# lmcinnes/enstop

Hardware: AMD Instinct MI355X
Metric: EM iterations/sec (higher is better)
Workload: dtype f32; 1 GPU; 1M x 100k, 100M nnz; corpus=independent Zipf tokens (SURVEY 8d), nnz=100435863, k=64, schedule=fused, parallelism=single fit

## Files before the change

### enstop_amd/csrc/plsa_hip.hip

```cpp
#include <hip/hip_runtime.h>
#include <hipcub/hipcub.hpp>
#include <rccl/rccl.h>

#include <algorithm>
#include <cmath>
#include <cstdarg>
#include <cstdio>
#include <cstdlib>
#include <cstring>
#include <memory>
#include <mutex>
#include <string>
#include <thread>
#include <type_traits>
#include <vector>

#include "../../include/plsa_hip.h"
#include "../../include/plsa_hip_diag.h"
#include "../../include/plsa_hip_members.h"
#include "../../include/plsa_hip_metrics.h"
#include "../../include/plsa_hip_blocked.h"
#include "../../include/plsa_hip_embed.h"
#include "../../include/plsa_hip_nmf.h"
#include "../../include/plsa_hip_score.h"
#include "../../include/plsa_hip_tempered.h"
#include "../../include/plsa_hip_online.h"
#include "mt_jump.hpp"
#include "plsa_embed_kernels.hpp"
#include "plsa_init_kernels.hpp"
#include "plsa_init_plan.hpp"
#include "plsa_kernels.hpp"
#include "plsa_launch_plan.hpp"
#include "plsa_member_kernels.hpp"
#include "plsa_metric_kernels.hpp"
#include "plsa_nmf_kernels.hpp"
#include "plsa_ref_kernels.hpp"
#include "plsa_synth.hpp"

using plsa::i64;

namespace {

thread_local std::string g_err;


struct DevBuf {
    void *p = nullptr;
    size_t cap = 0;
    bool borrowed = false;
    DevBuf() = default;
    DevBuf(DevBuf &&o) noexcept { swap(o); }
    DevBuf &operator=(DevBuf &&o) noexcept { DevBuf(std::move(o)).swap(*this); return *this; }
    void swap(DevBuf &o) noexcept { std::swap(p, o.p); std::swap(cap, o.cap); std::swap(borrowed, o.borrowed); }
    ~DevBuf() { if (p && !borrowed) (void)hipFree(p); }
    void release() { if (!borrowed) *this = DevBuf(); }
    void borrow(void *q, size_t bytes) { *this = DevBuf(); p = q; cap = q ? bytes : 0; borrowed = q != nullptr; }
    template <class T> T *as() const { return reinterpret_cast<T *>(p); }
};

template <class H, hipError_t (*Destroy)(H)>
struct Handle {
    H h = nullptr;
    Handle() = default;
    Handle(Handle &&o) noexcept { std::swap(h, o.h); }
    Handle &operator=(Handle &&o) noexcept { Handle(std::move(o)).swap(*this); return *this; }
    void swap(Handle &o) noexcept { std::swap(h, o.h); }
    ~Handle() { if (h) (void)Destroy(h); }
    operator H() const { return h; }
};
using Stream = Handle<hipStream_t, hipStreamDestroy>;
using Event = Handle<hipEvent_t, hipEventDestroy>;

struct HostFree { void operator()(void *p) const { (void)hipHostFree(p); } };
template <class T> using Pinned = std::unique_ptr<T[], HostFree>;
template <class T> hipError_t host_alloc(Pinned<T> &h, size_t count) {
    h.reset();
    void *q = nullptr;
    const hipError_t e = hipHostMalloc(&q, sizeof(T) * count, hipHostMallocDefault);
    h.reset(static_cast<T *>(q));
    return e;
}

template <class T> struct Derived {
    bool valid = false;
    void invalidate() { valid = false; }
    void drop() { static_cast<T &>(*this) = T{}; }
};

struct Timed {
    int name_id;
    Event a, b;
};

}

struct plsa_ctx {
    int device = 0;
    Stream stream;
    Stream stream2;
    hipStream_t ls = nullptr;
    Event ev_fork, ev_join;
    Event ev_row, ev_tail;
    bool overlap = true;
    double overlap_full_limit = 2e9;
    std::string err;
    hipDeviceProp_t prop;
    int grid_cap = 2048;

    i64 bn = 0, bm = 0, bnnz = 0;
    DevBuf b_indptr, b_col, b_val;
    bool active_is_base = true;
    i64 n = 0, m = 0, nnz = 0;
    DevBuf a_indptr, a_col, a_val;
    const int *indptr = nullptr, *col = nullptr;
    const float *val = nullptr;
    struct RowIndex : Derived<RowIndex> { DevBuf ids; } rowidx;

    struct Csc : Derived<Csc> {
        DevBuf colptr, row, val, pos, item_first, item_col, item_start, item_end, item_order, heavy_cols;
        DevBuf item_rec;
        DevBuf xcd_lo;
        bool balanced = false;
        int seg = 256, n_heavy = 0;
        i64 n_items = 0;
    } csc;
    int seg_override = 0, struct_lpn = 0;
    int struct_row_lpn = 0;
    DevBuf partial;
    bool use_item_order = true, xcd_split = true;
    bool packed = true;
    struct PackedStream : Derived<PackedStream> {
        DevBuf buf;
        bool ok = false;
        int state() const { return !valid ? -1 : (ok ? 1 : 0); }
    } pk_csr, pk_csc;
    DevBuf pk_count;
    int chunks_per_lane = 2;
    int row_lpn = 1, row_ch = 1;
    bool row_shape_8x2 = true;
    bool p_lent = false;
    int e_rows = -1;
    int mt_streams = 256;
    i64 mt_min_blocks = 4096;
    int heavy_items = 32;

    bool force_wide = false;
    struct RowItems : Derived<RowItems> {
        DevBuf first, row, start;
        bool use = false;
        int seg = 64;
        i64 n = 0;
    } ritems;
    int rseg_override = 0, ritems_mode = -1;
    DevBuf rpartial;

    struct EItems : Derived<EItems> { DevBuf row, start; int seg = 0; i64 n = 0; } eitems;
    int eseg_override = -1;

    bool sort_rows = true;
    struct RowOrder : Derived<RowOrder> {
        DevBuf ids;
        int range = 0;
    } roworder;
    i64 syn_n = 0; int syn_k0 = 0; double syn_alpha = 0.0; uint64_t syn_seed = 0;
    bool row_xcd = false;

    int k = 0, kp = 0, lpn = 1, ch = 1;
    DevBuf U[3], Vt[3], Vacc;
    bool rot3 = false;
    int speculate = -1;
    Event ev_ll;
    int cu = 0, cv = 0;
    i64 fac_n = 0, fac_m = 0;
    DevBuf P;
    struct PState : Derived<PState> {} p_state;
    bool ref_sums = false, ref_ll = false;
    DevBuf ref_terms;
    int ref_chain_mode = 0;
    bool ref_pairs_off = false;
    DevBuf ref_csum, ref_pairs, ref_exps, ref_pairs2, ref_exps2, ref_stats, ref_ll_neg;
    struct RefTileSums : Derived<RefTileSums> {
        DevBuf sums;
        const float *sw = nullptr;
        int tj = 0;
    } ref_tsum;
    const float *ref_e_sw = nullptr;
    bool ref_e_no_sums = false;
    struct RefHeavy : Derived<RefHeavy> { DevBuf cols; int n = 0, min = 0; } ref_heavy;
    int64_t p_budget = 0;
    struct RefBlocks : Derived<RefBlocks> {
        std::vector<i64> doc, ent;
        int64_t budget = 0;
        int kp = 0;
        i64 largest = 0;
        int blocks() const { return (int)doc.size() - 1; }
    } ref_blocks;
    struct PBlockInfo { int64_t budget = 0; int blocks = 0; int64_t largest = 0, p_bytes = 0; } p_block_info;
    Pinned<unsigned long long> h_ref_stats;
    Event ev_ref_stats;
    bool ref_stats_pending = false;
    unsigned long long ref_slow_total = 0, ref_chunks_total = 0;
    int placement_candidates = 4, placement_tried = 0;
    double placement_gbps[2] = {0.0, 0.0};
    size_t p_shift = 0;

    DevBuf sw, ll_partials, ll_out, colsum_partials, norm_pwz, norm_pdz, tmp0, tmp1, tmp2, cubtmp;
    DevBuf mt_seq;
    bool mt_chain = false;
    DevBuf mt_words, mt_state, mt_fin, mt_poly;
    Pinned<double> h_ll;

    DevBuf colsum_rows, colsum_rows2;
    DevBuf metric_mask, metric_small;
    struct Nmf { DevBuf raw, guarded, slabs, obj, out; } nmf;
    struct Score { DevBuf indptr, col, val, flag, out; } score;
    struct Tempered {
        DevBuf U, Vt, snapU, snapVt;
        bool have_snap = false;
        i64 snap_n = 0, snap_m = 0;
        int snap_k = 0;
    } tempered;
    DevBuf t_end;
    bool pipeline = true;
    bool graph = false;
    int order_band = -1;
    int balance = -1;
    bool bal_have_frac = false;
    double bal_frac[9] = {0, 0, 0, 0, 0, 0, 0, 0, 0};
    int bal_lo[9] = {0, 0, 0, 0, 0, 0, 0, 0, 0};
    i64 bal_chunks = -1;
    int bal_launches = 0;
    double bal_end_us[8] = {0, 0, 0, 0, 0, 0, 0, 0};
    int small_grid = 0;
    int colsum_rows_used = 0;
    struct FitInfo {
        int fused = 0, pipelined = 0, speculated = 0, graph_launches = 0;
        int tail = 0;
        int two_stage = 0;
        int xcd_split = 0;
    } fit_info;

    ncclComm_t comm = nullptr;
    int comm_rank = 0, comm_world = 1;
    bool sharded = false;
    bool sw_resident = false;
    i64 sw_n = 0;
    DevBuf sw_res;
    DevBuf comm_send, comm_recv, comm_small, comm_stack;
    Pinned<float> comm_host;
    size_t comm_host_cap = 0;

    bool timing = false;
    std::vector<std::string> names;
    std::vector<Timed> timed;
    std::vector<Event> pool;
    std::vector<double> acc_ms;
    std::vector<i64> acc_n;
};

namespace {

inline float *p_base(plsa_ctx *c) { return reinterpret_cast<float *>(reinterpret_cast<char *>(c->P.p) + c->p_shift); }

int fail(plsa_ctx *c, const char *fmt, ...) {
    char buf[512];
    va_list ap;
    va_start(ap, fmt);
    vsnprintf(buf, sizeof buf, fmt, ap);
    va_end(ap);
    if (c) c->err = buf; else g_err = buf;
    return 1;
}

#define HIPCHK(c, expr)                                                                            \
    do {                                                                                           \
        hipError_t e_ = (expr);                                                                    \
        if (e_ != hipSuccess)                                                                      \
            return fail((c), "%s failed: %s (%s:%d)", #expr, hipGetErrorString(e_), __FILE__,      \
                        __LINE__);                                                                 \
    } while (0)

#define CHK(expr)                                                                                  \
    do {                                                                                           \
        int r_ = (expr);                                                                           \
        if (r_) return r_;                                                                         \
    } while (0)
// ... 267 lines not shown

int launch_check(plsa_ctx *c, const char *what) {
    hipError_t e = hipGetLastError();
    if (e != hipSuccess) return fail(c, "launch of %s failed: %s", what, hipGetErrorString(e));
    return 0;
}

inline int out_u(const plsa_ctx *c) { return c->rot3 ? (c->cu + 1) % 3 : 1 - c->cu; }
inline int out_v(const plsa_ctx *c) { return c->rot3 ? (c->cv + 1) % 3 : 1 - c->cv; }

int grid_for(plsa_ctx *c, i64 work_items, int items_per_block) {
    return plsa::plan::grid_for(work_items, items_per_block, c->grid_cap);
}

}

#include "plsa_structures.hpp"

namespace {

int upload_sw(plsa_ctx *c, const float *sw, const float **d_sw) {
    *d_sw = nullptr;
    if (!sw) {
        if (c->sw_resident) {
            if (c->sw_n != c->n) return fail(c, "resident sample weights were set for %lld documents, the active matrix has %lld",
                                              (long long)c->sw_n, (long long)c->n);
            *d_sw = c->sw_res.as<float>();
        }
        return 0;
    }
    CHK(ensure(c, c->sw, sizeof(float) * (size_t)c->n));
    HIPCHK(c, hipMemcpyAsync(c->sw.p, sw, sizeof(float) * (size_t)c->n, hipMemcpyHostToDevice, c->stream));
    HIPCHK(c, hipStreamSynchronize(c->stream));
    *d_sw = c->sw.as<float>();
    return 0;
}

int need_factors(plsa_ctx *c) {
    if (c->k <= 0 || !c->U[0].p || !c->Vt[0].p) return fail(c, "factors not set (call plsa_set_factors)");
    if (c->n <= 0) return fail(c, "no corpus uploaded");
    if (c->fac_n != c->n || c->fac_m != c->m)
        return fail(c, "factors were set for a %lld x %lld matrix but the active matrix is %lld x %lld "
                       "(call plsa_set_factors after plsa_upload_csr / plsa_bootstrap)",
                    (long long)c->fac_n, (long long)c->fac_m, (long long)c->n, (long long)c->m);
    return 0;
}

template <class Fn> void with_flag(bool v, Fn &&fn) { if (v) fn(std::true_type{}); else fn(std::false_type{}); }
template <bool V, class Fn> void with_flag(std::integral_constant<bool, V> v, Fn &&fn) { fn(v); }

int ensure_p(plsa_ctx *c, i64 rows) {
    {
        const size_t need = sizeof(float) * (size_t)(rows + 64) * (size_t)c->kp;
        size_t free_b = 0, total_b = 0;
        if (!c->P.borrowed && c->P.cap < need && hipMemGetInfo(&free_b, &total_b) == hipSuccess && free_b + c->P.cap < need)
            return fail(c, c->ref_sums ? "the reference arithmetic (PLSA_REFERENCE_SUMS) stores P(z|w,d) like the reference does: %.1f GB needed, "
                                         "%.1f GB of HBM free -- at this size only the default arithmetic is available, or this one block "
                                         "of documents at a time (plsa_set_p_budget / p_budget=, plsa_fit and plsa_refit)"
                                       : "materialising P(z|w,d) needs %.1f GB but only %.1f GB of HBM are free; use the fused "
                           "schedule (PLSA_FUSED), which never stores it, or tile the documents (plsa_em_accumulate_materialised)", need / 1e9, (free_b + c->P.cap) / 1e9);
    }
    if (c->P.borrowed || c->p_lent) {
        const size_t need = sizeof(float) * (size_t)(rows + 64) * (size_t)c->kp;
        if (c->P.cap < need)
            return fail(c, c->P.borrowed ? "the borrowed P(z|w,d) buffer holds %.2f GB, this matrix needs %.2f GB (plsa_p_borrow)"
                                         : "the P(z|w,d) buffer lent out by plsa_p_reserve holds %.2f GB, this matrix needs %.2f GB: it cannot "
                                           "grow while other contexts hold its address (end the loans, then plsa_release_scratch)",
                        c->P.cap / 1e9, need / 1e9);
        c->p_shift = 0;
    } else
    {
        const char *s1 = getenv("PLSA_P_SLACK_MB"), *s2 = getenv("PLSA_P_OFFSET_KB");
        const bool budgeted = c->ref_sums && c->p_budget > 0;
        const size_t slack = s1 && !budgeted ? (size_t)atoll(s1) << 20 : 0;
        c->p_shift = s2 && !budgeted ? (size_t)atoll(s2) * 1024 : 0;
        CHK(ensure_best_placement(c, c->P, sizeof(float) * (size_t)(rows + 64) * (size_t)c->kp + std::max(slack, c->p_shift),
                                  budgeted ? 1 : c->placement_candidates, c->placement_gbps, &c->placement_tried));
    }
    return 0;
}

}

#include "plsa_ref.hpp"

namespace {

int run_e_step(plsa_ctx *c, float thresh) {
    c->ref_tsum.invalidate();
    CHK(ensure_p(c, c->nnz));
    if (c->ref_sums) return run_ref_e_step(c, thresh);
    bool e_rows = c->e_rows < 0 ? (double)c->nnz * c->kp >= 1e8 : c->e_rows != 0;
    if (e_rows) {
        const int eseg = plsa::plan::e_item_len(c->lpn, c->eseg_override);
        CHK(ensure_eitems(c, eseg));
        const bool items = eseg > 0 && c->eitems.n > 0;
        const int grid = grid_for(c, items ? c->eitems.n : c->n, 256 / c->lpn);
        const int *order = nullptr;
        if (!items) CHK(ensure_roworder(c, &order));
        CHK(dispatch_shape(c, [&](auto S) {
            Scope s(c, "k_e_step");
            auto go = [&](auto TN) {
                hipLaunchKernelGGL((plsa::k_e_step_rows<decltype(S), decltype(TN)::value>), dim3(grid), dim3(256), 0, c->stream,
                                   c->indptr, c->col, (int)c->n, order, c->U[c->cu].as<float>(), c->Vt[c->cv].as<float>(),
                                   p_base(c), c->kp, thresh, items ? c->eitems.row.as<int>() : nullptr,
                                   items ? c->eitems.start.as<int>() : nullptr, eseg, c->eitems.n);
            };
            if (thresh < plsa::TINY_THRESH) go(std::true_type{}); else go(std::false_type{});
        }));
    } else {
        CHK(ensure_rowidx(c));
        const i64 tiles = (c->nnz + 63) / 64;
        const int grid = grid_for(c, tiles, 4);
        CHK(dispatch_shape(c, [&](auto S) {
            Scope s(c, "k_e_step");
            auto go = [&](auto TN) {
                hipLaunchKernelGGL((plsa::k_e_step<decltype(S), decltype(TN)::value>), dim3(grid), dim3(256), 0, c->stream,
                                   c->rowidx.ids.as<int>(), c->col, c->nnz, c->U[c->cu].as<float>(),
                                   c->Vt[c->cv].as<float>(), p_base(c), c->kp, thresh);
            };
            if (thresh < plsa::TINY_THRESH) go(std::true_type{}); else go(std::false_type{});
        }));
    }
    CHK(launch_check(c, "k_e_step"));
    c->p_state.valid = true;
    return 0;
}

template <class Sh, class FromP, class Fn>
void select_row_pass(bool packed, FromP from_p, bool want_ll, bool tiny, Fn &&fn) {
    with_flag(from_p, [&](auto FP) {
        if constexpr (decltype(FP)::value) fn(Sh{}, FP, std::false_type{}, std::false_type{});
        else with_flag(want_ll, [&](auto LL) {
            with_flag(tiny, [&](auto TN) { if (packed) fn(plsa::Packed<Sh>{}, FP, LL, TN); else fn(Sh{}, FP, LL, TN); });
        });
    });
}

template <class Sh, class FromP, class Timed, class Fn>
void select_col_pass(bool packed, FromP from_p, Timed timed, bool tiny, Fn &&fn) {
    with_flag(from_p, [&](auto FP) {
        with_flag(timed, [&](auto TM) {
            if constexpr (decltype(FP)::value) fn(Sh{}, FP, TM, std::false_type{});
            else with_flag(tiny, [&](auto TN) { if (packed) fn(plsa::Packed<Sh>{}, FP, TM, TN); else fn(Sh{}, FP, TM, TN); });
        });
    });
}

struct RowLaunch {
    plsa::plan::RowPass plan;
    bool items, packed, xcd_rows;
    const int *indptr, *colidx;
    const float *vals;
    const int *order;
    const int *ritem_row, *ritem_start, *ritem_first;
    float *rpartial;
    double *ll_partials;
    i64 n_ritems;
    int rseg;
};

int prepare_row_pass(plsa_ctx *c, bool from_p, bool want_ll, RowLaunch &r) {
    CHK(ensure_ritems(c));
    r.items = c->ritems.use && c->ritems.n > 0;
    r.xcd_rows = !r.items && !from_p && c->sort_rows && row_xcd_range(c) > 0;
    r.plan = plsa::plan::row_pass(c->n, c->ritems.n, r.items, c->row_lpn, c->grid_cap, r.xcd_rows);
    r.order = nullptr;
    if (!r.items) CHK(ensure_roworder(c, &r.order));
    if (r.items) CHK(ensure(c, c->rpartial, sizeof(float) * (size_t)c->ritems.n * c->kp));
    if (want_ll) CHK(ensure(c, c->ll_partials, sizeof(double) * (size_t)r.plan.grid));
    if (!from_p) CHK(ensure_packed_csr(c));
    r.packed = !from_p && c->packed && c->pk_csr.ok;
    r.indptr = c->indptr; r.colidx = r.packed ? c->pk_csr.buf.as<int>() : c->col; r.vals = c->val;
    r.ritem_row = r.items ? c->ritems.row.as<int>() : nullptr;
    r.ritem_start = r.items ? c->ritems.start.as<int>() : nullptr;
    r.ritem_first = r.items ? c->ritems.first.as<int>() : nullptr;
    r.rpartial = r.items ? c->rpartial.as<float>() : nullptr;
    r.ll_partials = c->ll_partials.as<double>();
    r.n_ritems = c->ritems.n; r.rseg = c->ritems.seg;
    return 0;
}

int run_row_pass(plsa_ctx *c, bool from_p, bool want_ll, const float *d_sw, float thresh,
                 float *d_norm_pdz, int *ll_blocks) {
    RowLaunch r;
    CHK(prepare_row_pass(c, from_p, want_ll, r));
    CHK(dispatch_shape_row(c, [&](auto S) {
        using Sh = decltype(S);
        const float *U = c->U[c->cu].as<float>(), *Vt = c->Vt[c->cv].as<float>();
        float *Un = c->U[out_u(c)].as<float>();
        const int n = (int)c->n, kp = c->kp;
        select_row_pass<Sh>(r.packed, from_p, want_ll, thresh < plsa::TINY_THRESH, [&](auto SS, auto FP, auto LL, auto TN) {
            Scope s(c, from_p ? "k_row_pass<P>" : want_ll ? "k_row_pass<fused,LL>" : "k_row_pass<fused>");
            hipLaunchKernelGGL((plsa::k_row_pass<decltype(SS), decltype(FP)::value, decltype(LL)::value, decltype(TN)::value>),
                               dim3(r.plan.grid), dim3(256), 0, c->ls, r.indptr, r.colidx, r.vals, n, r.order, U, Vt, p_base(c), Un,
                               d_sw, d_norm_pdz, kp, thresh, r.ll_partials, r.ritem_row, r.ritem_start, r.rseg, r.n_ritems,
                               r.rpartial, r.xcd_rows ? 1 : 0);
        });
        if (r.items) {
            Scope s(c, "k_row_reduce");
            hipLaunchKernelGGL((plsa::k_row_reduce<Sh>), dim3(r.plan.reduce_grid), dim3(256), 0, c->ls,
                               r.ritem_first, n, r.rpartial, Un, d_norm_pdz, kp);
        }
    }));
    CHK(launch_check(c, "k_row_pass"));
    if (ll_blocks) *ll_blocks = r.plan.grid;
    return 0;
}

struct ColLaunch {
    plsa::plan::ColPass plan;
    bool packed;
    int xcd_split;
    const int4 *item_rec;
    i64 n_items;
    const int *csc_row, *csc_pos;
    const float *csc_val;
    float *partial;
    double *colsum_rows, *colsum_rows2;
    float *norm_pwz;
    const int *item_first, *heavy_cols;
    int n_heavy, heavy_items;
};

int prepare_col_pass(plsa_ctx *c, bool from_p, ColLaunch &l) {
    CHK(from_p ? ensure_csc(c) : ensure_packed_csc(c));
    l.packed = !from_p && c->packed && c->pk_csc.ok;
    l.plan = plsa::plan::col_pass(c->csc.n_items, c->m, c->lpn, c->csc.n_heavy, c->grid_cap);
    l.xcd_split = plsa::plan::xcd_split(c->xcd_split, l.plan.n_chunks, c->n, c->kp) ? 1 : 0;
    CHK(ensure(c, c->partial, sizeof(float) * (size_t)std::max<i64>(c->csc.n_items, 1) * c->kp));
    CHK(ensure(c, c->colsum_rows, sizeof(double) * (size_t)std::max(l.plan.n_chunks, 1) * c->kp));
    CHK(ensure(c, c->norm_pwz, sizeof(float) * (size_t)c->kp));
    if (l.plan.norm_blocks) CHK(ensure(c, c->colsum_rows2, sizeof(double) * (size_t)l.plan.norm_blocks * c->kp));
    l.item_rec = c->csc.item_rec.as<int4>(); l.n_items = c->csc.n_items;
    l.csc_row = l.packed ? c->pk_csc.buf.as<int>() : c->csc.row.as<int>();
    l.csc_pos = c->csc.pos.as<int>(); l.csc_val = c->csc.val.as<float>();
    l.partial = c->partial.as<float>(); l.norm_pwz = c->norm_pwz.as<float>();
    l.colsum_rows = c->colsum_rows.as<double>(); l.colsum_rows2 = c->colsum_rows2.as<double>();
    l.item_first = c->csc.item_first.as<int>(); l.heavy_cols = c->csc.heavy_cols.as<int>();
    l.n_heavy = c->csc.n_heavy; l.heavy_items = c->heavy_items;
    return 0;
}

int run_col_pass(plsa_ctx *c, bool from_p, const float *d_sw, float thresh, int parts = 3) {
    ColLaunch l;
    CHK(prepare_col_pass(c, from_p, l));
    int rc = 0;
    CHK(dispatch_shape_gather(c, table_is_wide(c, c->n), [&](auto S) {
        using Sh = decltype(S);
        constexpr int GPB = 256 / Sh::LPN;
        const int n_chunks = l.plan.n_chunks, kp = c->kp;
        if (parts & 1) {
            c->fit_info.xcd_split = l.xcd_split;
            const size_t smem = sizeof(double) * (size_t)GPB * kp;
            auto launch = [&](bool timed) -> int {
                int grid = plsa::plan::col_grid(c->bal_lo, n_chunks, l.xcd_split != 0);
                if (c->small_grid > 0 && (double)c->nnz * kp < c->overlap_full_limit)
                    grid = std::min(grid, c->small_grid * c->prop.multiProcessorCount);
                Scope s(c, from_p ? "k_col_pass<P>" : "k_col_pass<fused>");
                const int *lo = c->csc.xcd_lo.as<int>();
                const float *U = c->U[c->cu].as<float>(), *Vt = c->Vt[c->cv].as<float>();
                unsigned long long *te = c->t_end.as<unsigned long long>();
                select_col_pass<Sh>(l.packed, from_p, timed, thresh < plsa::TINY_THRESH, [&](auto SS, auto FP, auto TM, auto TN) {
                    hipLaunchKernelGGL((plsa::k_col_pass<decltype(SS), decltype(FP)::value, decltype(TM)::value, decltype(TN)::value>),
                                       dim3(grid), dim3(256), smem, c->ls, l.item_rec, l.n_items, lo, l.csc_row, l.csc_val, l.csc_pos,
                                       U, Vt, p_base(c), d_sw, l.partial, kp, thresh, l.xcd_split, l.colsum_rows, te);
                });
                return launch_check(c, "k_col_pass");
            };
            rc = ensure_balance(c, n_chunks, l.xcd_split != 0, launch);
            if (rc) return;
            rc = launch(false);
            if (rc) return;
            c->colsum_rows_used = n_chunks;
        }
        if (parts & 2) {
            Scope s(c, "k_col_reduce");
            hipLaunchKernelGGL((plsa::k_col_reduce<Sh>), dim3(l.plan.reduce_grid), dim3(256), GPB * kp * sizeof(float), c->ls,
                               l.item_first, (int)c->m, l.heavy_items, l.heavy_cols, l.n_heavy, l.partial, c->Vacc.as<float>(), kp);
        }
    }));
    if (rc) return rc;
    CHK(launch_check(c, "k_col_pass"));
    return 0;
}

int run_v_normalise(plsa_ctx *c) {
    if (c->sharded && c->comm) {
        Scope s(c, "rccl_allreduce_accumulator");
        NCCLCHK(c, ncclAllReduce(c->Vacc.p, c->Vacc.p, (size_t)c->m * c->kp, ncclFloat, ncclSum, c->comm, c->ls));
    }
    const int nb = (int)std::min<i64>(plsa::NORM_BLOCKS, std::max<i64>(1, c->m));
    CHK(ensure(c, c->colsum_partials, sizeof(double) * (size_t)nb * c->kp));
    {
        Scope s(c, "k_colsum_partial");
        hipLaunchKernelGGL(plsa::k_colsum_partial, dim3(nb), dim3(256), 256 * sizeof(double), c->ls,
                           c->Vacc.as<float>(), (int)c->m, c->kp, c->colsum_partials.as<double>());
    }
    CHK(ensure(c, c->norm_pwz, sizeof(float) * (size_t)c->kp));
    {
        Scope s(c, "k_colsum_final");
        hipLaunchKernelGGL(plsa::k_colsum_final, dim3(1), dim3(256), 0, c->ls,
                           c->colsum_partials.as<double>(), nb, c->kp, c->norm_pwz.as<float>());
    }
    {
        Scope s(c, "k_v_normalise");
        const i64 total4 = c->m * c->kp / 4;
        hipLaunchKernelGGL(plsa::k_v_normalise, dim3(grid_for(c, total4, 256)), dim3(256),
                           c->kp * sizeof(float), c->ls, c->Vacc.as<float>(),
                           c->Vt[out_v(c)].as<float>(), (int)c->m, c->kp, c->norm_pwz.as<float>());
    }
    CHK(launch_check(c, "k_v_normalise"));
    return 0;
}

int run_col_tail(plsa_ctx *c) {
    if (c->sharded) {
        c->fit_info.tail = 2;
        c->fit_info.two_stage = 0;
        CHK(run_col_pass(c, false, nullptr, 0.f, 2));
        return run_v_normalise(c);
    }
    ColLaunch l;
    CHK(prepare_col_pass(c, true, l));
    c->fit_info.tail = 1;
    c->fit_info.two_stage = l.plan.norm_blocks > 0;
    if (c->colsum_rows_used <= 0) return fail(c, "internal: column tail without a column pass");
    const double *rows_in = l.colsum_rows;
    int n_rows = l.plan.n_chunks;
    if (l.plan.norm_blocks) {
        Scope s(c, "k_norm_reduce");
        hipLaunchKernelGGL(plsa::k_norm_reduce, dim3(l.plan.norm_blocks), dim3(256), 0, c->ls, rows_in, n_rows, c->kp,
                           l.colsum_rows2);
        rows_in = l.colsum_rows2;
        n_rows = l.plan.norm_blocks;
    }
    {
        Scope s(c, "k_colsum_final");
        hipLaunchKernelGGL(plsa::k_colsum_final, dim3(1), dim3(256), 0, c->ls, rows_in, n_rows, c->kp, l.norm_pwz);
    }
    CHK(dispatch_shape(c, [&](auto S) {
        using Sh = decltype(S);
        constexpr int GPB = 256 / Sh::LPN;
        Scope s(c, "k_col_reduce_norm");
        hipLaunchKernelGGL((plsa::k_col_reduce_norm<Sh>), dim3(l.plan.reduce_grid), dim3(256),
                           sizeof(float) * (size_t)(GPB + 1) * c->kp, c->ls, l.item_first, (int)c->m, l.heavy_items, l.heavy_cols,
                           l.n_heavy, l.partial, l.norm_pwz, c->Vt[out_v(c)].as<float>(), c->kp);
    }));
    return launch_check(c, "k_col_reduce_norm");
}

int finish_ll(plsa_ctx *c, int blocks, double *out) {
    CHK(ensure(c, c->ll_out, sizeof(double)));
    {
        Scope s(c, "k_ll_final");
        hipLaunchKernelGGL(plsa::k_ll_final, dim3(1), dim3(256), 0, c->stream,
                           c->ll_partials.as<double>(), blocks, c->ll_out.as<double>());
    }
    CHK(launch_check(c, "k_ll_final"));
    if (c->sharded && c->comm)
        NCCLCHK(c, ncclAllReduce(c->ll_out.p, c->ll_out.p, 1, ncclDouble, ncclSum, c->comm, c->stream));
    HIPCHK(c, hipMemcpyAsync(c->h_ll.get(), c->ll_out.p, sizeof(double), hipMemcpyDeviceToHost, c->stream));
    if (!out) return hipEventRecord(c->ev_ll, c->stream) == hipSuccess ? 0 : fail(c, "event record failed");
    HIPCHK(c, hipStreamSynchronize(c->stream));
    *out = c->h_ll[0];
    return 0;
}

int wait_ll(plsa_ctx *c, double *out) {
    HIPCHK(c, hipEventSynchronize(c->ev_ll));
    *out = c->h_ll[0];
    return 0;
}

int run_loglik(plsa_ctx *c, const float *d_sw, double *out) {
    if (c->ref_ll) return run_ref_loglik(c, d_sw, out);
    const int grid = grid_for(c, c->n, 256 / c->lpn);
    const int *order = nullptr;
    CHK(ensure_roworder(c, &order));
    CHK(ensure(c, c->ll_partials, sizeof(double) * (size_t)grid));
    CHK(dispatch_shape(c, [&](auto S) {
        Scope s(c, "k_loglik");
        hipLaunchKernelGGL((plsa::k_loglik<decltype(S)>), dim3(grid), dim3(256), 0, c->stream, c->indptr,
                           c->col, c->val, (int)c->n, order, c->U[c->cu].as<float>(),
                           c->Vt[c->cv].as<float>(), d_sw, c->kp, c->ll_partials.as<double>());
    }));
    CHK(launch_check(c, "k_loglik"));
    return finish_ll(c, grid, out);
}

int run_m_step_from_p(plsa_ctx *c, const float *d_sw, bool update_v, float *d_norm_pdz) {
    if (!c->p_state.valid) return fail(c, "plsa_m_step: no P(z|w,d) on the device (run plsa_e_step or plsa_set_p)");
    if (c->ref_sums) return run_ref_m_step(c, d_sw, update_v, d_norm_pdz);
    CHK(run_row_pass(c, true, false, nullptr, 0.f, d_norm_pdz, nullptr));
    if (update_v) {
        CHK(run_col_pass(c, true, d_sw, 0.f, 1));
        CHK(run_col_tail(c));
    }
    c->cu ^= 1;
    if (update_v) c->cv ^= 1;
    return 0;
}

void read_knobs(plsa_ctx *c) {
    if (const char *s = getenv("PLSA_OVERLAP")) c->overlap = atoi(s) != 0;
    if (const char *s = getenv("PLSA_OVERLAP_FULL_LIMIT")) c->overlap_full_limit = atof(s);
    if (const char *s = getenv("PLSA_ROW_ITEMS")) c->ritems_mode = atoi(s);
    if (const char *s = getenv("PLSA_PACKED")) c->packed = atoi(s) != 0;
    if (const char *s = getenv("PLSA_ROW_SEG")) c->rseg_override = std::max(1, atoi(s));
    int mult = 128;
    if (const char *s = getenv("PLSA_GRID_MULT")) mult = std::max(1, atoi(s));
    c->grid_cap = c->prop.multiProcessorCount * mult;
    if (const char *s = getenv("PLSA_CONTIG")) g_contig = atoi(s) != 0;
    if (const char *s = getenv("PLSA_PLACEMENT_CANDIDATES")) c->placement_candidates = std::max(1, atoi(s));
    if (const char *s = getenv("PLSA_COL_SEG")) c->seg_override = std::max(1, atoi(s));
    if (const char *s = getenv("PLSA_HEAVY_ITEMS")) c->heavy_items = std::max(1, atoi(s));
    if (const char *s = getenv("PLSA_SORT_ROWS")) c->sort_rows = atoi(s) != 0;
    if (const char *s = getenv("PLSA_ROW_XCD")) c->row_xcd = atoi(s) != 0;
// ... 1111 lines not shown
```

### enstop_amd/csrc/plsa_kernels.hpp

```cpp
#pragma once
#include <hip/hip_runtime.h>
#include <stdint.h>

#ifndef PLSA_UNR
#define PLSA_UNR 4
#endif
#ifndef PLSA_NT_STREAMS
#define PLSA_NT_STREAMS 0
#endif
#ifndef PLSA_UNR_E
#define PLSA_UNR_E 16
#endif
#ifndef PLSA_WAVES
#define PLSA_WAVES 1
#endif
#ifndef PLSA_UNR_COL
#define PLSA_UNR_COL 8
#endif
#ifndef PLSA_WAVES_COL
#define PLSA_WAVES_COL PLSA_WAVES
#endif

namespace plsa {

typedef long long i64;
typedef unsigned long long u64;

template <int CTRL>
__device__ __forceinline__ float dpp_mov(float v) {
    return __int_as_float(__builtin_amdgcn_update_dpp(0, __float_as_int(v), CTRL, 0xF, 0xF, true));
}

template <int LPN>
__device__ __forceinline__ float group_sum(float v) {
    if (LPN >= 2) v += dpp_mov<0xB1>(v);
    if (LPN >= 4) v += dpp_mov<0x4E>(v);
    if (LPN >= 8) v += dpp_mov<0x141>(v);
    if (LPN >= 16) v += dpp_mov<0x140>(v);
    if (LPN >= 32) v += __shfl_xor(v, 16, 64);
    if (LPN >= 64) v += __shfl_xor(v, 32, 64);
    return v;
}

__device__ __forceinline__ float hsum(const float4 &a) { return (a.x + a.y) + (a.z + a.w); }
__device__ __forceinline__ float hsum_products(const float4 &a) {
#pragma clang fp contract(off)
    return (a.x + a.y) + (a.z + a.w);
}
__device__ __forceinline__ float4 zero4() { return make_float4(0.f, 0.f, 0.f, 0.f); }

__device__ __forceinline__ float4 ld4(const float *p) { return *reinterpret_cast<const float4 *>(p); }
__device__ __forceinline__ void st4(float *p, const float4 &v) { *reinterpret_cast<float4 *>(p) = v; }
typedef float f4v __attribute__((ext_vector_type(4)));
__device__ __forceinline__ void st4_nt(float *p, const float4 &v) {
    f4v t = {v.x, v.y, v.z, v.w};
    __builtin_nontemporal_store(t, reinterpret_cast<f4v *>(p));
}
__device__ __forceinline__ float4 ld4_nt(const float *p) {
    const f4v t = __builtin_nontemporal_load(reinterpret_cast<const f4v *>(p));
    return make_float4(t.x, t.y, t.z, t.w);
}

__device__ __forceinline__ int ldi(const int *p) { return PLSA_NT_STREAMS ? __builtin_nontemporal_load(p) : *p; }
__device__ __forceinline__ float ldf(const float *p) { return PLSA_NT_STREAMS ? __builtin_nontemporal_load(p) : *p; }

template <int LPN_, int CH_, bool FULL_, bool WIDE_ = false>
struct Shape {
    static constexpr int LPN = LPN_, CH = CH_;
    static constexpr bool FULL = FULL_, WIDE = WIDE_;
    static constexpr int UNR = (LPN_ <= 8 && CH_ == 1) ? LPN_ : ((LPN_ < PLSA_UNR) ? LPN_ : PLSA_UNR);
    static constexpr int UNR_COL = (LPN_ < PLSA_UNR_COL) ? LPN_ : PLSA_UNR_COL;
    static constexpr int UNR_EF = (LPN_ < 4) ? LPN_ : 4;
    static constexpr int UNR_E_CAP = (PLSA_UNR_E / CH_ > 0) ? PLSA_UNR_E / CH_ : 1;
    static constexpr int UNR_E = (LPN_ < UNR_E_CAP) ? LPN_ : UNR_E_CAP;
    __device__ static __forceinline__ int kp(int kp_rt) { return FULL_ ? 4 * LPN_ * CH_ : kp_rt; }
    __device__ static __forceinline__ int c4(int li, int j) { return 4 * (li + LPN_ * j); }
    __device__ static __forceinline__ bool ok(int li, int j, int kp) { return FULL_ || c4(li, j) < kp; }
    static constexpr bool PACKED = false;
};

template <class S>
struct Packed : S {
    static constexpr bool PACKED = true;
};
constexpr long long PACK_MAX_IDS = 1ll << 24;
__device__ __forceinline__ unsigned pack_code(float v) {
    return (v >= 1.f && v <= 255.f && v == truncf(v)) ? (unsigned)v : 0u;
}
__device__ __forceinline__ void unpack_entry(int &id, float &x, const float *__restrict__ vals, int j, int j_end) {
    const unsigned e = (unsigned)id;
    id = (int)(e & 0xFFFFFFu);
    x = (float)(e >> 24);
    if (x == 0.f && j < j_end) x = ldf(vals + j);
}

template <class S, bool ZERO_INVALID, bool STREAM = false>
__device__ __forceinline__ void load_row(const float *row, int li, int kp, float4 (&out)[S::CH]) {
#pragma unroll
    for (int j = 0; j < S::CH; ++j) {
        const bool ok = S::ok(li, j, kp);
        const float *p = row + (ok ? S::c4(li, j) : 0);
        const float4 v = STREAM ? ld4_nt(p) : ld4(p);
        out[j] = (ZERO_INVALID && !ok) ? zero4() : v;
    }
}

template <class S>
__device__ __forceinline__ void gather_row(const float *table, int row, int li, int kp, float4 (&out)[S::CH]) {
    if constexpr (S::WIDE) {
        load_row<S, false>(table + (i64)row * kp, li, kp, out);
    } else {
        const unsigned base = (unsigned)row * (unsigned)(kp * 4);
#pragma unroll
        for (int j = 0; j < S::CH; ++j) {
            const unsigned off = S::ok(li, j, kp) ? base + 4u * (unsigned)S::c4(li, j) : base;
            out[j] = *reinterpret_cast<const float4 *>(reinterpret_cast<const char *>(table) + off);
        }
    }
}

template <int CH, bool WANT_UNTH>
__device__ __forceinline__ float products(const float4 (&u)[CH], const float4 (&vt)[CH],
                                          float thresh, float4 (&keep)[CH], float &unth) {
    float part = 0.f;
    unth = 0.f;
#pragma unroll
    for (int j = 0; j < CH; ++j) {
        float4 v;
        v.x = vt[j].x * u[j].x; v.y = vt[j].y * u[j].y; v.z = vt[j].z * u[j].z; v.w = vt[j].w * u[j].w;
        if (WANT_UNTH) unth = j ? unth + hsum_products(v) : hsum_products(v);
        keep[j].x = v.x > thresh ? v.x : 0.f;
        keep[j].y = v.y > thresh ? v.y : 0.f;
        keep[j].z = v.z > thresh ? v.z : 0.f;
        keep[j].w = v.w > thresh ? v.w : 0.f;
        part = j ? part + hsum(keep[j]) : hsum(keep[j]);
    }
    return part;
}

__device__ __forceinline__ float inv_norm(float norm) {
    return norm > 0.f ? __builtin_amdgcn_rcpf(norm) : 0.f;
}

template <int CH>
__device__ __forceinline__ void scale(float4 (&a)[CH], float s) {
#pragma unroll
    for (int j = 0; j < CH; ++j) { a[j].x *= s; a[j].y *= s; a[j].z *= s; a[j].w *= s; }
}

constexpr float TINY_THRESH = 5e-38f;
template <int CH>
__device__ __forceinline__ void rescue_tiny(bool tiny, float &norm, float4 (&keep)[CH]) {
    if (tiny && norm < 0x1p-100f) {
        norm *= 0x1p100f;
        scale(keep, 0x1p100f);
    }
}

template <class S, bool TINY = false>
__global__ __launch_bounds__(256, PLSA_WAVES) void k_e_step(const int *__restrict__ rowidx,
                                                const int *__restrict__ colidx, i64 nnz,
                                                const float *__restrict__ U,
                                                const float *__restrict__ Vt, float *__restrict__ P,
                                                int kp_rt, float thresh) {
    constexpr int LPN = S::LPN, CH = S::CH, UNR = S::UNR_EF;
    constexpr int GPW = 64 / LPN;
    const int kp = S::kp(kp_rt);
    const int lane = threadIdx.x & 63;
    const int wave = threadIdx.x >> 6;
    const int g = lane / LPN, li = lane % LPN;
    const i64 tiles = (nnz + 63) >> 6;
    constexpr bool tiny = TINY;
    for (i64 t = (i64)blockIdx.x * 4 + wave; t < tiles; t += (i64)gridDim.x * 4) {
        const i64 base = t << 6;
        const i64 mine = base + lane;
        const int d_l = mine < nnz ? __builtin_nontemporal_load(rowidx + mine) : 0;
        const int w_l = mine < nnz ? __builtin_nontemporal_load(colidx + mine) : 0;
#pragma unroll
        for (int s0 = 0; s0 < LPN; s0 += UNR) {
            float4 u[UNR][CH], vt[UNR][CH];
#pragma unroll
            for (int q = 0; q < UNR; ++q) {
                const int src = (s0 + q) * GPW + g;
                const int d = __shfl(d_l, src, 64);
                const int w = __shfl(w_l, src, 64);
                load_row<S, true, PLSA_NT_STREAMS>(U + (i64)d * kp, li, kp, u[q]);
                load_row<S, false>(Vt + (i64)w * kp, li, kp, vt[q]);
            }
#pragma unroll
            for (int q = 0; q < UNR; ++q) {
                float4 keep[CH];
                float unth;
                float norm = group_sum<LPN>(products<CH, false>(u[q], vt[q], thresh, keep, unth));
                rescue_tiny(tiny, norm, keep);
                const float inv = inv_norm(norm);
                float *prow = P + (base + (s0 + q) * GPW + g) * kp;
#pragma unroll
                for (int j = 0; j < CH; ++j) {
                    if (S::ok(li, j, kp)) {
                        float4 p;
                        p.x = keep[j].x * inv; p.y = keep[j].y * inv;
                        p.z = keep[j].z * inv; p.w = keep[j].w * inv;
                        st4_nt(prow + S::c4(li, j), p);
                    }
                }
            }
        }
    }
}

template <class S, bool TINY = false>
__global__ __launch_bounds__(256, PLSA_WAVES) void k_e_step_rows(const int *__restrict__ indptr,
                                                     const int *__restrict__ colidx, int n,
                                                     const int *__restrict__ row_order,
                                                     const float *__restrict__ U,
                                                     const float *__restrict__ Vt, float *__restrict__ P,
                                                     int kp_rt, float thresh,
                                                     const int *__restrict__ ritem_row,
                                                     const int *__restrict__ ritem_start, int rseg,
                                                     i64 n_ritems) {
    constexpr int LPN = S::LPN, CH = S::CH, UNR = S::UNR_E;
    constexpr int GPB = 256 / LPN;
    const int kp = S::kp(kp_rt);
    const int li = threadIdx.x % LPN;
    const int gid = threadIdx.x / LPN;
    const bool items = ritem_row != nullptr;
    const i64 n_work = items ? n_ritems : (i64)n;
    constexpr bool tiny = TINY;
    for (i64 r = (i64)blockIdx.x * GPB + gid; r < n_work; r += (i64)gridDim.x * GPB) {
        const int d = items ? ritem_row[r] : (row_order ? row_order[r] : (int)r);
        const int j0 = items ? ritem_start[r] : indptr[d];
        const int j1 = items ? min(j0 + rseg, indptr[d + 1]) : indptr[d + 1];
        float4 u[CH];
        load_row<S, true, PLSA_NT_STREAMS>(U + (i64)d * kp, li, kp, u);
        int w_n = (j0 + li < j1) ? ldi(colidx + j0 + li) : 0;
        for (int jb = j0; jb < j1; jb += LPN) {
            const int w_l = w_n;
            const int jn = jb + LPN + li;
            w_n = jn < j1 ? ldi(colidx + jn) : 0;
            const int cnt = min(LPN, j1 - jb);
            for (int s0 = 0; s0 < cnt; s0 += UNR) {
                float4 vt[UNR][CH];
#pragma unroll
                for (int q = 0; q < UNR; ++q)
                    load_row<S, false>(Vt + (i64)__shfl(w_l, s0 + q, LPN) * kp, li, kp, vt[q]);
#pragma unroll
                for (int q = 0; q < UNR; ++q) {
                    float4 keep[CH];
                    float unth;
                    float norm = group_sum<LPN>(products<CH, false>(u, vt[q], thresh, keep, unth));
                    rescue_tiny(tiny, norm, keep);
                    const float inv = inv_norm(norm);
                    if (s0 + q < cnt) {
                        float *prow = P + (i64)(jb + s0 + q) * kp;
#pragma unroll
                        for (int j = 0; j < CH; ++j) {
                            if (S::ok(li, j, kp)) {
                                float4 p;
                                p.x = keep[j].x * inv; p.y = keep[j].y * inv;
                                p.z = keep[j].z * inv; p.w = keep[j].w * inv;
                                st4_nt(prow + S::c4(li, j), p);
                            }
                        }
                    }
                }
            }
        }
    }
}

template <class S, bool FROM_P, bool WANT_LL, bool TINY>
__device__ __forceinline__ void row_pass_body(const int *__restrict__ indptr,
                                                  const int *__restrict__ colidx,
                                                  const float *__restrict__ vals, int n,
                                                  const int *__restrict__ row_order,
                                                  const float *__restrict__ U,
                                                  const float *__restrict__ Vt,
                                                  const float *__restrict__ P,
                                                  float *__restrict__ U_new,
                                                  const float *__restrict__ sw,
                                                  float *__restrict__ norm_pdz_out, int kp_rt,
                                                  float thresh, double *__restrict__ ll_partials,
                                                  const int *__restrict__ ritem_row,
                                                  const int *__restrict__ ritem_start, int rseg,
                                                  i64 n_ritems, float *__restrict__ rpartial, int xcd_rows, unsigned block, unsigned nblocks) {
    constexpr int LPN = S::LPN, CH = S::CH, UNR = S::UNR;
    constexpr int GPB = 256 / LPN;
    const int kp = S::kp(kp_rt);
    const int li = threadIdx.x % LPN;
    const int gid = threadIdx.x / LPN;
    double ll = 0.0;
    const i64 first_block = xcd_rows ? (i64)(block & 7) * (nblocks >> 3) + (block >> 3) : (i64)block;
    constexpr bool tiny = !FROM_P && TINY;
    const bool items = ritem_row != nullptr;
    const i64 n_work = items ? n_ritems : (i64)n;
    for (i64 r = first_block * GPB + gid; r < n_work; r += (i64)nblocks * GPB) {
        const int d = items ? ritem_row[r] : (row_order ? row_order[r] : (int)r);
        const int j0 = items ? ritem_start[r] : indptr[d];
        const int j1 = items ? min(j0 + rseg, indptr[d + 1]) : indptr[d + 1];
        float4 u[CH], acc[CH];
        load_row<S, true, PLSA_NT_STREAMS>(U + (i64)d * kp, li, kp, u);
#pragma unroll
        for (int j = 0; j < CH; ++j) acc[j] = zero4();
        const float swd = (WANT_LL && sw) ? sw[d] : 1.0f;
        int w_n = (j0 + li < j1) ? ldi(colidx + j0 + li) : 0;
        float x_n = (!S::PACKED && j0 + li < j1) ? ldf(vals + j0 + li) : 0.f;
        for (int jb = j0; jb < j1; jb += LPN) {
            int w_l = w_n;
            float x_l = x_n;
            if (S::PACKED) unpack_entry(w_l, x_l, vals, jb + li, j1);
            const int jn = jb + LPN + li;
            w_n = jn < j1 ? ldi(colidx + jn) : 0;
            if (!S::PACKED) x_n = jn < j1 ? ldf(vals + jn) : 0.f;
            const int cnt = min(LPN, j1 - jb);
            for (int s0 = 0; s0 < cnt; s0 += UNR) {
                float4 a[UNR][CH];
                float x[UNR];
                constexpr bool OWNER = !FROM_P && UNR == LPN;
#pragma unroll
                for (int q = 0; q < UNR; ++q) {
                    const int w = __shfl(w_l, s0 + q, LPN);
                    if (!OWNER) x[q] = __shfl(x_l, s0 + q, LPN);
                    if (FROM_P) load_row<S, false>(P + (i64)min(jb + s0 + q, j1 - 1) * kp, li, kp, a[q]);
                    else gather_row<S>(Vt, w, li, kp, a[q]);
                }
                float my_dot = 1.f, my_x = 0.f;
                if (OWNER) {
                    float nmine = 0.f;
#pragma unroll
                    for (int q = 0; q < UNR; ++q) {
                        float unth;
                        const float part = products<CH, WANT_LL>(u, a[q], thresh, a[q], unth);
                        float norm = group_sum<LPN>(part);
                        rescue_tiny(tiny, norm, a[q]);
                        if (WANT_LL) {
                            const float dot = group_sum<LPN>(unth);
                            if (li == q && s0 + q < cnt) { my_dot = dot; my_x = x_l; }
                        }
                        nmine = (li == s0 + q) ? norm : nmine;
                    }
                    const float xs_mine = x_l * inv_norm(nmine);
#pragma unroll
                    for (int q = 0; q < UNR; ++q) {
                        const float xs = __shfl(xs_mine, s0 + q, LPN);
#pragma unroll
                        for (int j = 0; j < CH; ++j) {
                            acc[j].x += xs * a[q][j].x; acc[j].y += xs * a[q][j].y;
                            acc[j].z += xs * a[q][j].z; acc[j].w += xs * a[q][j].w;
                        }
                    }
                } else {
#pragma unroll
                for (int q = 0; q < UNR; ++q) {
                    float4 pz[CH];
                    if (FROM_P) {
#pragma unroll
                        for (int j = 0; j < CH; ++j) pz[j] = S::ok(li, j, kp) ? a[q][j] : zero4();
                    } else {
                        float unth;
                        const float part = products<CH, WANT_LL>(u, a[q], thresh, pz, unth);
                        float norm = group_sum<LPN>(part);
                        rescue_tiny(tiny, norm, pz);
                        if (WANT_LL) {
                            const float dot = group_sum<LPN>(unth);
                            if (li == q && s0 + q < cnt) { my_dot = dot; my_x = x[q]; }
                        }
                        x[q] *= inv_norm(norm);
                    }
#pragma unroll
                    for (int j = 0; j < CH; ++j) {
                        acc[j].x += x[q] * pz[j].x; acc[j].y += x[q] * pz[j].y;
                        acc[j].z += x[q] * pz[j].z; acc[j].w += x[q] * pz[j].w;
                    }
                }
                }
                if (WANT_LL && !FROM_P && li < UNR) ll += (double)(my_x * logf(my_dot) * swd);
            }
        }
        if (items) {
#pragma unroll
            for (int j = 0; j < CH; ++j)
                if (S::ok(li, j, kp)) st4(rpartial + r * kp + S::c4(li, j), acc[j]);
            continue;
        }
        float part = 0.f;
#pragma unroll
        for (int j = 0; j < CH; ++j) part += hsum(acc[j]);
        const float rown = group_sum<LPN>(part);
        if (norm_pdz_out && li == 0) norm_pdz_out[d] = rown;
#pragma unroll
        for (int j = 0; j < CH; ++j) {
            if (S::ok(li, j, kp)) {
                float4 o = acc[j];
                if (rown > 0.f) { o.x /= rown; o.y /= rown; o.z /= rown; o.w /= rown; }
                st4(U_new + (i64)d * kp + S::c4(li, j), o);
            }
        }
    }
    if (WANT_LL) {
        __shared__ double red[256];
        red[threadIdx.x] = ll;
        __syncthreads();
        for (int s = 128; s > 0; s >>= 1) {
            if ((int)threadIdx.x < s) red[threadIdx.x] += red[threadIdx.x + s];
            __syncthreads();
        }
        if (threadIdx.x == 0) ll_partials[block] = red[0];
    }
}

template <class S, bool FROM_P, bool WANT_LL, bool TINY = false>
__global__ __launch_bounds__(256, PLSA_WAVES) void k_row_pass(const int *__restrict__ indptr,
                                                  const int *__restrict__ colidx,
                                                  const float *__restrict__ vals, int n,
                                                  const int *__restrict__ row_order,
                                                  const float *__restrict__ U,
                                                  const float *__restrict__ Vt,
                                                  const float *__restrict__ P,
                                                  float *__restrict__ U_new,
                                                  const float *__restrict__ sw,
                                                  float *__restrict__ norm_pdz_out, int kp_rt,
                                                  float thresh, double *__restrict__ ll_partials,
                                                  const int *__restrict__ ritem_row,
                                                  const int *__restrict__ ritem_start, int rseg,
                                                  i64 n_ritems, float *__restrict__ rpartial, int xcd_rows) {
    row_pass_body<S, FROM_P, WANT_LL, TINY>(indptr, colidx, vals, n, row_order, U, Vt, P, U_new, sw, norm_pdz_out, kp_rt, thresh,
                                            ll_partials, ritem_row, ritem_start, rseg, n_ritems, rpartial, xcd_rows,
                                            blockIdx.x, gridDim.x);
}

template <class S>
__device__ __forceinline__ void row_reduce_body(const int *__restrict__ ritem_first, int n,
                                                const float *__restrict__ rpartial,
                                                float *__restrict__ U_new,
                                                float *__restrict__ norm_pdz_out, int kp_rt, unsigned block, unsigned nblocks) {
    constexpr int LPN = S::LPN, CH = S::CH;
    constexpr int GPB = 256 / LPN;
    const int kp = S::kp(kp_rt);
    const int li = threadIdx.x % LPN;
    const int gid = threadIdx.x / LPN;
    for (i64 d = (i64)block * GPB + gid; d < n; d += (i64)nblocks * GPB) {
        const int i0 = ritem_first[d], i1 = ritem_first[d + 1];
        float4 acc[CH];
#pragma unroll
        for (int j = 0; j < CH; ++j) acc[j] = zero4();
        for (int it = i0; it < i1; ++it) {
            float4 p[CH];
            load_row<S, true>(rpartial + (i64)it * kp, li, kp, p);
#pragma unroll
            for (int j = 0; j < CH; ++j) {
                acc[j].x += p[j].x; acc[j].y += p[j].y; acc[j].z += p[j].z; acc[j].w += p[j].w;
            }
        }
        float part = 0.f;
#pragma unroll
        for (int j = 0; j < CH; ++j) part += hsum(acc[j]);
        const float rown = group_sum<LPN>(part);
        if (norm_pdz_out && li == 0) norm_pdz_out[d] = rown;
#pragma unroll
        for (int j = 0; j < CH; ++j) {
            if (S::ok(li, j, kp)) {
                float4 o = acc[j];
                if (rown > 0.f) { o.x /= rown; o.y /= rown; o.z /= rown; o.w /= rown; }
                st4(U_new + d * kp + S::c4(li, j), o);
            }
        }
    }
}

template <class S>
__global__ __launch_bounds__(256) void k_row_reduce(const int *__restrict__ ritem_first, int n,
                                                    const float *__restrict__ rpartial,
                                                    float *__restrict__ U_new,
                                                    float *__restrict__ norm_pdz_out, int kp_rt) {
    row_reduce_body<S>(ritem_first, n, rpartial, U_new, norm_pdz_out, kp_rt, blockIdx.x, gridDim.x);
}

__global__ void k_ritem_fill(const int *__restrict__ indptr, const int *__restrict__ ritem_first, int n,
                             int seg, int *__restrict__ ritem_row, int *__restrict__ ritem_start) {
    const i64 d = (i64)blockIdx.x * blockDim.x + threadIdx.x;
    if (d < n) {
        const int i0 = ritem_first[d], i1 = ritem_first[d + 1];
        for (int i = i0; i < i1; ++i) {
            ritem_row[i] = (int)d;
            ritem_start[i] = indptr[d] + (i - i0) * seg;
        }
    }
}

template <class S, int THREADS = 256>
__device__ __forceinline__ void block_colsum(const float4 (&csum)[S::CH], int li, int gid, int kp,
                                             double *sred , double *__restrict__ out_row) {
    constexpr int GPB = THREADS / S::LPN;
#pragma unroll
    for (int j = 0; j < S::CH; ++j) {
        if (S::ok(li, j, kp)) {
            double *p = sred + gid * kp + S::c4(li, j);
            p[0] = (double)csum[j].x; p[1] = (double)csum[j].y; p[2] = (double)csum[j].z; p[3] = (double)csum[j].w;
        }
    }
    __syncthreads();
    for (int z = threadIdx.x; z < kp; z += THREADS) {
        double t = 0.0;
        for (int g = 0; g < GPB; ++g) t += sred[g * kp + z];
        out_row[z] = t;
    }
}

template <class S, bool FROM_P, int UN, bool TINY>
__device__ __forceinline__ void col_batch(int s0, int d_l, float x_l, int p_l, int li, int kp, float thresh,
                                          const float *__restrict__ U, const float *__restrict__ P,
                                          const float4 (&vt)[S::CH], float4 (&acc)[S::CH]) {
    constexpr int LPN = S::LPN, CH = S::CH;
    constexpr bool OWNER = !FROM_P && UN >= 4;
    float4 a[UN][CH];
    float x[UN];
#pragma unroll
    for (int q = 0; q < UN; ++q) {
        if (!OWNER) x[q] = __shfl(x_l, s0 + q, LPN);
        if (FROM_P) {
            const int pos = __shfl(p_l, s0 + q, LPN);
            load_row<S, false>(P + (i64)pos * kp, li, kp, a[q]);
        } else {
            const int d = __shfl(d_l, s0 + q, LPN);
            gather_row<S>(U, d, li, kp, a[q]);
        }
    }
    if (OWNER) {
        float nmine = 0.f;
#pragma unroll
        for (int q = 0; q < UN; ++q) {
            float unth;
            float norm = group_sum<LPN>(products<CH, false>(a[q], vt, thresh, a[q], unth));
            rescue_tiny(TINY, norm, a[q]);
            nmine = (li == s0 + q) ? norm : nmine;
        }
        const float xs_mine = x_l * inv_norm(nmine);
#pragma unroll
        for (int q = 0; q < UN; ++q) {
            const float xs = __shfl(xs_mine, s0 + q, LPN);
#pragma unroll
            for (int j = 0; j < CH; ++j) {
                acc[j].x += xs * a[q][j].x; acc[j].y += xs * a[q][j].y;
                acc[j].z += xs * a[q][j].z; acc[j].w += xs * a[q][j].w;
            }
        }
        return;
    }
#pragma unroll
    for (int q = 0; q < UN; ++q) {
        float4 pz[CH];
        if (FROM_P) {
#pragma unroll
            for (int j = 0; j < CH; ++j) pz[j] = S::ok(li, j, kp) ? a[q][j] : zero4();
        } else {
            float unth;
            float norm = group_sum<LPN>(products<CH, false>(a[q], vt, thresh, pz, unth));
            rescue_tiny(TINY, norm, pz);
            x[q] *= inv_norm(norm);
        }
#pragma unroll
        for (int j = 0; j < CH; ++j) {
            acc[j].x += x[q] * pz[j].x; acc[j].y += x[q] * pz[j].y;
            acc[j].z += x[q] * pz[j].z; acc[j].w += x[q] * pz[j].w;
        }
    }
}

template <class S, bool FROM_P, bool TIMED, bool TINY>
__device__ __forceinline__ void col_pass_body(const int4 *__restrict__ item_rec, i64 n_items,
                                                  const int *__restrict__ xcd_lo,
                                                  const int *__restrict__ csc_row,
                                                  const float *__restrict__ csc_val,
                                                  const int *__restrict__ csc_pos,
                                                  const float *__restrict__ U,
                                                  const float *__restrict__ Vt,
                                                  const float *__restrict__ P,
                                                  const float *__restrict__ sw,
                                                  float *__restrict__ partial, int kp_rt, float thresh,
                                                  int xcd_split, double *__restrict__ chunk_sums,
                                                  unsigned long long *__restrict__ t_end, double *scol , unsigned block, unsigned nblocks) {
    constexpr int LPN = S::LPN, CH = S::CH, UNR = S::UNR_COL;
    constexpr int GPB = 256 / LPN;
    const int kp = S::kp(kp_rt);
    const int li = threadIdx.x % LPN;
    const int gid = threadIdx.x / LPN;
    const int n_chunks = (int)((n_items + GPB - 1) / GPB);
    const int xcd = xcd_split ? (int)(block & 7) : 0;
    const int nq = xcd_split ? (int)((nblocks + 7 - xcd) / 8) : (int)nblocks;
    const int q = xcd_split ? (int)(block >> 3) : (int)block;
    const int c_lo = xcd_split ? xcd_lo[xcd] : 0, c_hi = xcd_split ? xcd_lo[xcd + 1] : n_chunks;
    if (TIMED && block == 0 && threadIdx.x == 0) t_end[nblocks] = wall_clock64();
    for (int chunk = c_lo + q; chunk < c_hi; chunk += nq) {
        const i64 io = (i64)chunk * GPB + gid;
        float4 acc[CH];
#pragma unroll
        for (int j = 0; j < CH; ++j) acc[j] = zero4();
        if (io < n_items) {
            const int4 rec = item_rec[io];
            const int w = rec.x, j0 = rec.y, j1 = rec.z;
            float4 vt[CH];
            load_row<S, true, PLSA_NT_STREAMS>(Vt + (i64)w * kp, li, kp, vt);
            int d_n = (j0 + li < j1) ? ldi(csc_row + j0 + li) : 0;
            float x_n = (!S::PACKED && j0 + li < j1) ? ldf(csc_val + j0 + li) : 0.f;
            int p_n = (FROM_P && j0 + li < j1) ? ldi(csc_pos + j0 + li) : 0;
            for (int jb = j0; jb < j1; jb += LPN) {
                int d_l = d_n;
                const int p_l = p_n;
                float x_l = x_n;
                if (S::PACKED) unpack_entry(d_l, x_l, csc_val, jb + li, j1);
                const int jn = jb + LPN + li;
                d_n = jn < j1 ? ldi(csc_row + jn) : 0;
                if (!S::PACKED) x_n = jn < j1 ? ldf(csc_val + jn) : 0.f;
                if (FROM_P) p_n = jn < j1 ? ldi(csc_pos + jn) : 0;
                if (sw) x_l *= sw[d_l];
                const int cnt = min(LPN, j1 - jb);
                int s0 = 0;
                for (; s0 + UNR <= cnt; s0 += UNR)
                    col_batch<S, FROM_P, UNR, TINY>(s0, d_l, x_l, p_l, li, kp, thresh, U, P, vt, acc);
                constexpr int TAIL = (UNR >= 2 && LPN >= 2) ? 2 : 1;
                for (; s0 < cnt; s0 += TAIL)
                    col_batch<S, FROM_P, TAIL, TINY>(s0, d_l, x_l, p_l, li, kp, thresh, U, P, vt, acc);
            }
#pragma unroll
            for (int j = 0; j < CH; ++j)
                if (S::ok(li, j, kp)) st4(partial + (i64)rec.w * kp + S::c4(li, j), acc[j]);
        }
        block_colsum<S>(acc, li, gid, kp, scol, chunk_sums + (i64)chunk * kp);
        __syncthreads();
    }
    if (TIMED && threadIdx.x == 0) t_end[block] = wall_clock64();
}

template <class S, bool FROM_P, bool TIMED, bool TINY = false>
__global__ __launch_bounds__(256, PLSA_WAVES_COL) void k_col_pass(const int4 *__restrict__ item_rec, i64 n_items,
                                                  const int *__restrict__ xcd_lo,
                                                  const int *__restrict__ csc_row,
                                                  const float *__restrict__ csc_val,
                                                  const int *__restrict__ csc_pos,
                                                  const float *__restrict__ U,
                                                  const float *__restrict__ Vt,
                                                  const float *__restrict__ P,
                                                  const float *__restrict__ sw,
                                                  float *__restrict__ partial, int kp_rt, float thresh,
                                                  int xcd_split, double *__restrict__ chunk_sums,
                                                  unsigned long long *__restrict__ t_end) {
    extern __shared__ double scol[];
    col_pass_body<S, FROM_P, TIMED, TINY>(item_rec, n_items, xcd_lo, csc_row, csc_val, csc_pos, U, Vt, P, sw, partial, kp_rt, thresh,
                                          xcd_split, chunk_sums, t_end, scol, blockIdx.x, gridDim.x);
}

__global__ void k_item_records(const int *__restrict__ item_order, const int *__restrict__ item_col,
                               const int *__restrict__ item_start, const int *__restrict__ item_end, i64 n_items,
                               int4 *__restrict__ rec) {
    const i64 io = (i64)blockIdx.x * blockDim.x + threadIdx.x;
    if (io < n_items) {
        const int it = item_order ? item_order[io] : (int)io;
        rec[io] = make_int4(item_col[it], item_start[it], item_end[it], it);
    }
}

__device__ __forceinline__ float div_pos(float v, float n) { return n > 0.f ? v / n : v; }

template <class S, bool NORMALISE>
__device__ __forceinline__ void col_reduce_body(const int *__restrict__ item_first, int m, int heavy_items,
                                                const int *__restrict__ heavy_cols, int n_heavy,
                                                const float *__restrict__ partial, float *__restrict__ Vt_new,
                                                int kp, int block, int nblocks, float *sacc ,
                                                const float *snorm ) {
    constexpr int LPN = S::LPN, CH = S::CH;
    constexpr int GPB = 256 / LPN;
    const int li = threadIdx.x % LPN;
    const int gid = threadIdx.x / LPN;
    float4 acc[CH];
    for (int h = block; h < n_heavy; h += nblocks) {
        const int c = heavy_cols[h];
        const int i0 = item_first[c], i1 = item_first[c + 1];
#pragma unroll
        for (int j = 0; j < CH; ++j) acc[j] = zero4();
        constexpr int B = 4;
        for (int it = i0 + gid; it < i1; it += GPB * B) {
            float4 p[B][CH];
#pragma unroll
            for (int u = 0; u < B; ++u) {
                const int iu = it + u * GPB;
                if (iu < i1) {
                    load_row<S, true>(partial + (i64)iu * kp, li, kp, p[u]);
                } else {
#pragma unroll
                    for (int j = 0; j < CH; ++j) p[u][j] = zero4();
                }
            }
#pragma unroll
            for (int u = 0; u < B; ++u)
#pragma unroll
                for (int j = 0; j < CH; ++j) {
                    acc[j].x += p[u][j].x; acc[j].y += p[u][j].y; acc[j].z += p[u][j].z; acc[j].w += p[u][j].w;
                }
        }
#pragma unroll
        for (int j = 0; j < CH; ++j)
            if (S::ok(li, j, kp)) st4(sacc + gid * kp + S::c4(li, j), acc[j]);
        __syncthreads();
        for (int z = threadIdx.x; z < kp; z += 256) {
            float t = 0.f;
            for (int g = 0; g < GPB; ++g) t += sacc[g * kp + z];
            Vt_new[(i64)c * kp + z] = NORMALISE ? div_pos(t, snorm[z]) : t;
        }
        __syncthreads();
    }
    for (i64 c = (i64)block * GPB + gid; c < m; c += (i64)nblocks * GPB) {
        const int i0 = item_first[c], i1 = item_first[c + 1];
        if (i1 - i0 > heavy_items) continue;
#pragma unroll
        for (int j = 0; j < CH; ++j) acc[j] = zero4();
        int it = i0;
        for (; it + 4 <= i1; it += 4) {
            float4 p[4][CH];
#pragma unroll
            for (int u = 0; u < 4; ++u) load_row<S, true>(partial + (i64)(it + u) * kp, li, kp, p[u]);
#pragma unroll
            for (int u = 0; u < 4; ++u)
#pragma unroll
                for (int j = 0; j < CH; ++j) {
                    acc[j].x += p[u][j].x; acc[j].y += p[u][j].y; acc[j].z += p[u][j].z; acc[j].w += p[u][j].w;
                }
        }
        for (; it < i1; ++it) {
            float4 p[CH];
            load_row<S, true>(partial + (i64)it * kp, li, kp, p);
#pragma unroll
            for (int j = 0; j < CH; ++j) {
                acc[j].x += p[j].x; acc[j].y += p[j].y; acc[j].z += p[j].z; acc[j].w += p[j].w;
            }
        }
#pragma unroll
        for (int j = 0; j < CH; ++j) {
            if (S::ok(li, j, kp)) {
                float4 o = acc[j];
                if (NORMALISE) {
                    const float *nn = snorm + S::c4(li, j);
                    o.x = div_pos(o.x, nn[0]); o.y = div_pos(o.y, nn[1]); o.z = div_pos(o.z, nn[2]); o.w = div_pos(o.w, nn[3]);
                }
                st4(Vt_new + c * kp + S::c4(li, j), o);
            }
        }
    }
}

template <class S>
__global__ __launch_bounds__(256) void k_col_reduce(const int *__restrict__ item_first, int m,
                                                    int heavy_items, const int *__restrict__ heavy_cols,
                                                    int n_heavy, const float *__restrict__ partial,
                                                    float *__restrict__ Vt_new, int kp_rt) {
    extern __shared__ float sacc[];
    col_reduce_body<S, false>(item_first, m, heavy_items, heavy_cols, n_heavy, partial, Vt_new, S::kp(kp_rt),
                              (int)blockIdx.x, (int)gridDim.x, sacc, nullptr);
}

template <class S>
__global__ __launch_bounds__(256) void k_col_reduce_norm(const int *__restrict__ item_first, int m,
                                                         int heavy_items, const int *__restrict__ heavy_cols,
                                                         int n_heavy, const float *__restrict__ partial,
                                                         const float *__restrict__ norm_pwz,
                                                         float *__restrict__ Vt_out, int kp_rt) {
    extern __shared__ float sdyn[];
    const int kp = S::kp(kp_rt);
    constexpr int GPB = 256 / S::LPN;
    float *snorm = sdyn + GPB * kp;
    for (int z = threadIdx.x; z < kp; z += 256) snorm[z] = norm_pwz[z];
    __syncthreads();
    col_reduce_body<S, true>(item_first, m, heavy_items, heavy_cols, n_heavy, partial, Vt_out, kp,
                             (int)blockIdx.x, (int)gridDim.x, sdyn, snorm);
}

__global__ void k_heavy_list(const int *__restrict__ item_first, int m, int heavy_items,
                             int *__restrict__ heavy_cols, int *__restrict__ n_heavy) {
    const i64 c = (i64)blockIdx.x * blockDim.x + threadIdx.x;
    if (c < m && item_first[c + 1] - item_first[c] > heavy_items)
        heavy_cols[atomicAdd(n_heavy, 1)] = (int)c;
}

constexpr int NORM_BLOCKS = 256;

__device__ __forceinline__ void colsum_slab_body(const float *__restrict__ Vt_new, int m, int kp, int slab,
                                                 int n_slabs, double *__restrict__ partials, double *sred ) {
    const i64 per = ((i64)m + n_slabs - 1) / n_slabs;
    const i64 w0 = (i64)slab * per, w1 = min((i64)m, w0 + per);
    for (int zb = 0; zb < kp; zb += 256) {
        const int span = min(256, kp - zb);
        const int rpp = 256 / span;
        const int z = zb + (int)threadIdx.x % span;
        const int ro = (int)threadIdx.x / span;
        float s = 0.f;
        if (ro < rpp)
            for (i64 w = w0 + ro; w < w1; w += rpp) s += Vt_new[w * kp + z];
        sred[threadIdx.x] = (ro < rpp) ? (double)s : 0.0;
        __syncthreads();
        if ((int)threadIdx.x < span) {
            double tot = 0.0;
            for (int r = 0; r < rpp; ++r) tot += sred[r * span + threadIdx.x];
// ... 110 lines not shown

__global__ void k_ll_final(const double *__restrict__ partials, int nb, double *__restrict__ out) {
    __shared__ double red[256];
    ll_final_body(partials, nb, out, red);
}

template <class S>
__global__ __launch_bounds__(256, PLSA_WAVES) void k_loglik(const int *__restrict__ indptr,
                                                const int *__restrict__ colidx,
                                                const float *__restrict__ vals, int n,
                                                const int *__restrict__ row_order,
                                                const float *__restrict__ U,
                                                const float *__restrict__ Vt,
                                                const float *__restrict__ sw, int kp_rt,
                                                double *__restrict__ ll_partials) {
    constexpr int LPN = S::LPN, CH = S::CH, UNR = S::UNR;
    constexpr int GPB = 256 / LPN;
    const int kp = S::kp(kp_rt);
    const int li = threadIdx.x % LPN;
    const int gid = threadIdx.x / LPN;
    double ll = 0.0;
    for (i64 r = (i64)blockIdx.x * GPB + gid; r < n; r += (i64)gridDim.x * GPB) {
        const int d = row_order ? row_order[r] : (int)r;
        const int j0 = indptr[d], j1 = indptr[d + 1];
        float4 u[CH];
        load_row<S, true, PLSA_NT_STREAMS>(U + (i64)d * kp, li, kp, u);
        const float swd = sw ? sw[d] : 1.0f;
        int w_n = (j0 + li < j1) ? ldi(colidx + j0 + li) : 0;
        float x_n = (j0 + li < j1) ? ldf(vals + j0 + li) : 0.f;
        for (int jb = j0; jb < j1; jb += LPN) {
            const int w_l = w_n;
            const float x_l = x_n;
            const int jn = jb + LPN + li;
            w_n = jn < j1 ? ldi(colidx + jn) : 0;
            x_n = jn < j1 ? ldf(vals + jn) : 0.f;
            const int cnt = min(LPN, j1 - jb);
            for (int s0 = 0; s0 < cnt; s0 += UNR) {
                float4 vt[UNR][CH];
                float x[UNR];
#pragma unroll
                for (int q = 0; q < UNR; ++q) {
                    const int w = __shfl(w_l, s0 + q, LPN);
                    x[q] = __shfl(x_l, s0 + q, LPN);
                    load_row<S, false>(Vt + (i64)w * kp, li, kp, vt[q]);
                }
#pragma unroll
                for (int q = 0; q < UNR; ++q) {
                    float part = 0.f;
#pragma unroll
                    for (int j = 0; j < CH; ++j)
                        part += (vt[q][j].x * u[j].x + vt[q][j].y * u[j].y) + (vt[q][j].z * u[j].z + vt[q][j].w * u[j].w);
                    const float dot = group_sum<LPN>(part);
                    if (li == 0 && s0 + q < cnt) ll += (double)(x[q] * logf(dot) * swd);
                }
            }
        }
    }
    __shared__ double red[256];
    red[threadIdx.x] = ll;
    __syncthreads();
    for (int s = 128; s > 0; s >>= 1) {
        if ((int)threadIdx.x < s) red[threadIdx.x] += red[threadIdx.x + s];
        __syncthreads();
    }
    if (threadIdx.x == 0) ll_partials[blockIdx.x] = red[0];
}

__global__ void k_expand_rows(const int *__restrict__ indptr, int n, int *__restrict__ rowidx) {
    const int lane = threadIdx.x & 63;
    const i64 wid = ((i64)blockIdx.x * blockDim.x + threadIdx.x) >> 6;
    const i64 nw = ((i64)gridDim.x * blockDim.x) >> 6;
    for (i64 d = wid; d < n; d += nw) {
        const int j0 = indptr[d], j1 = indptr[d + 1];
        for (int j = j0 + lane; j < j1; j += 64) rowidx[j] = (int)d;
    }
}

__global__ void k_row_lengths(const int *__restrict__ indptr, int n, int *__restrict__ len,
                              int *__restrict__ ids, int range) {
    const i64 r = (i64)blockIdx.x * blockDim.x + threadIdx.x;
    if (r < n) {
        const int l = indptr[r + 1] - indptr[r];
        len[r] = range > 0 ? (int)((unsigned)((n - 1) / range - (int)(r / range)) << 22 | (unsigned)min(l, (1 << 22) - 1)) : l;
        ids[r] = (int)r;
    }
}

__global__ void k_validate_csr(const int *__restrict__ indptr, const int *__restrict__ indices, i64 n, i64 m, i64 nnz,
                               int *__restrict__ bad) {
    int b = 0;
    const i64 stride = (i64)gridDim.x * blockDim.x;
    for (i64 i = (i64)blockIdx.x * blockDim.x + threadIdx.x; i < n; i += stride) {
        const int a = indptr[i], e = indptr[i + 1];
        if (a > e || a < 0 || (i64)e > nnz) b |= 1;
    }
    for (i64 j = (i64)blockIdx.x * blockDim.x + threadIdx.x; j < nnz; j += stride) {
        const int w = indices[j];
        if (w < 0 || (i64)w >= m) b |= 2;
    }
    if (b) atomicOr(bad, b);
}

__global__ void k_boot_lengths(const int *__restrict__ base_indptr, const i64 *__restrict__ idx,
                               i64 n_out, i64 n_base, int *__restrict__ lens, int *__restrict__ bad) {
    const i64 i = (i64)blockIdx.x * blockDim.x + threadIdx.x;
    if (i < n_out) {
        const i64 r = idx[i];
        if (r < 0 || r >= n_base) { lens[i] = 0; atomicOr(bad, 1); }
        else lens[i] = base_indptr[r + 1] - base_indptr[r];
    }
}

__global__ void k_boot_gather(const int *__restrict__ base_indptr, const int *__restrict__ base_col,
                              const float *__restrict__ base_val, const i64 *__restrict__ idx,
                              i64 n_out, const i64 *__restrict__ out_ptr64,
                              int *__restrict__ out_indptr, int *__restrict__ out_col,
                              float *__restrict__ out_val) {
    const int lane = threadIdx.x & 63;
    const i64 wid = ((i64)blockIdx.x * blockDim.x + threadIdx.x) >> 6;
    const i64 nw = ((i64)gridDim.x * blockDim.x) >> 6;
    for (i64 i = wid; i <= n_out; i += nw) {
        if (lane == 0) out_indptr[i] = (int)out_ptr64[i];
        if (i == n_out) break;
        const i64 r = idx[i];
        const int s0 = base_indptr[r], len = base_indptr[r + 1] - s0;
        const i64 o0 = out_ptr64[i];
        for (int j = lane; j < len; j += 64) {
            out_col[o0 + j] = base_col[s0 + j];
            out_val[o0 + j] = base_val[s0 + j];
        }
    }
}

__global__ void k_iota(int *__restrict__ a, i64 nn) {
    for (i64 i = (i64)blockIdx.x * blockDim.x + threadIdx.x; i < nn; i += (i64)gridDim.x * blockDim.x)
        a[i] = (int)i;
}
__global__ void k_colptr_from_sorted(const int *__restrict__ keys_sorted, i64 nnz, int m,
                                     int *__restrict__ colptr) {
    const i64 w = (i64)blockIdx.x * blockDim.x + threadIdx.x;
    if (w > m) return;
    i64 lo = 0, hi = nnz;
    while (lo < hi) {
        const i64 mid = (lo + hi) >> 1;
        if (keys_sorted[mid] < (int)w) lo = mid + 1; else hi = mid;
    }
    colptr[w] = (int)lo;
}

__device__ __forceinline__ void add_escapes(unsigned esc, unsigned long long *__restrict__ n_esc) {
    for (int o = 32; o > 0; o >>= 1) esc += __shfl_xor(esc, o, 64);
    if ((threadIdx.x & 63) == 0 && esc) atomicAdd(n_esc, (unsigned long long)esc);
}
__global__ __launch_bounds__(256) void k_pack_entries(const int *__restrict__ ids, const float *__restrict__ vals, i64 nnz,
                                                      unsigned *__restrict__ packed, unsigned long long *__restrict__ n_esc) {
    unsigned esc = 0;
    for (i64 i = (i64)blockIdx.x * blockDim.x + threadIdx.x; i < nnz; i += (i64)gridDim.x * blockDim.x) {
        const unsigned code = pack_code(vals[i]);
        packed[i] = (unsigned)ids[i] | (code << 24);
        esc += code == 0u;
    }
    add_escapes(esc, n_esc);
}
__global__ __launch_bounds__(256) void k_csc_gather(const int *__restrict__ pos, const int *__restrict__ rowidx,
                                                    const float *__restrict__ vals, i64 nnz, int *__restrict__ csc_row,
                                                    float *__restrict__ csc_val, unsigned *__restrict__ packed,
                                                    unsigned long long *__restrict__ n_esc) {
    unsigned esc = 0;
    for (i64 i = (i64)blockIdx.x * blockDim.x + threadIdx.x; i < nnz; i += (i64)gridDim.x * blockDim.x) {
        const int p = pos[i];
        const int r = rowidx[p];
        const float v = vals[p];
        csc_row[i] = r;
        csc_val[i] = v;
        if (packed) {
            const unsigned code = pack_code(v);
            packed[i] = (unsigned)r | (code << 24);
            esc += code == 0u;
        }
    }
    if (packed) add_escapes(esc, n_esc);
}
__global__ void k_item_counts(const int *__restrict__ colptr, int m, int seg, int *__restrict__ cnt) {
    const i64 c = (i64)blockIdx.x * blockDim.x + threadIdx.x;
    if (c < m) cnt[c] = (colptr[c + 1] - colptr[c] + seg - 1) / seg;
}

__global__ void k_item_fill(const int *__restrict__ colptr, const int *__restrict__ item_first, int m, int seg,
                            const int *__restrict__ csc_row, int *__restrict__ item_col,
                            int *__restrict__ item_start, int *__restrict__ item_end, int band, int len_bits,
                            unsigned long long *__restrict__ item_key, int *__restrict__ item_id, int n_items) {
    const i64 i = (i64)blockIdx.x * blockDim.x + threadIdx.x;
    if (i >= n_items) return;
    int lo = 0, hi = m;
    while (hi - lo > 1) {
        const int mid = (lo + hi) >> 1;
        if (item_first[mid] <= (int)i) lo = mid; else hi = mid;
    }
    const int c = lo;
    const int st = colptr[c] + ((int)i - item_first[c]) * seg;
    item_col[i] = c;
    item_start[i] = st;
    item_end[i] = min(st + seg, colptr[c + 1]);
    const unsigned first = (unsigned)csc_row[st];
    const unsigned long long inv_len = ((1ull << len_bits) - 1ull) - (unsigned long long)(colptr[c + 1] - colptr[c]);
    item_key[i] = band > 0 ? ((unsigned long long)(first / (unsigned)band) << len_bits) | inv_len
                           : (unsigned long long)first;
    item_id[i] = (int)i;
}

template <bool NT>
__global__ __launch_bounds__(256) void k_probe_fill(float *__restrict__ p, i64 n4) {
    const float4 v = make_float4(1.f, 2.f, 3.f, 4.f);
    for (i64 i = (i64)blockIdx.x * 256 + threadIdx.x; i < n4; i += (i64)gridDim.x * 256) {
        if (NT) st4_nt(p + i * 4, v); else st4(p + i * 4, v);
    }
}
__global__ __launch_bounds__(256) void k_probe_fill_tiled(float *__restrict__ p, i64 n4, int rows) {
    const float4 v = make_float4(1.f, 2.f, 3.f, 4.f);
    const int lane = threadIdx.x & 63, wave = threadIdx.x >> 6;
    const i64 tiles = n4 / (64 * (i64)rows);
    for (i64 t = (i64)blockIdx.x * 4 + wave; t < tiles; t += (i64)gridDim.x * 4) {
        float *base = p + (t * rows * 64 + lane) * 4;
        for (int r = 0; r < rows; ++r) st4_nt(base + (i64)r * 256, v);
    }
}
__global__ __launch_bounds__(256) void k_probe_read(const float *__restrict__ a, float *__restrict__ sink, i64 n4) {
    float4 acc = zero4();
    for (i64 i = (i64)blockIdx.x * 256 + threadIdx.x; i < n4; i += (i64)gridDim.x * 256) {
        const float4 v = ld4(a + i * 4);
        acc.x += v.x; acc.y += v.y; acc.z += v.z; acc.w += v.w;
    }
    if (acc.x + acc.y + acc.z + acc.w == -1.2345f) sink[0] = acc.x;
}
__global__ __launch_bounds__(256) void k_probe_copy(const float *__restrict__ a, float *__restrict__ b, i64 n4) {
    for (i64 i = (i64)blockIdx.x * 256 + threadIdx.x; i < n4; i += (i64)gridDim.x * 256)
        st4(b + i * 4, ld4(a + i * 4));
}

__global__ __launch_bounds__(256) void k_hell_prepare(float *__restrict__ R, int t, i64 m, double *__restrict__ l1) {
    __shared__ double red[256];
    const int i = blockIdx.x;
    float *row = R + (i64)i * m;
    double s = 0.0;
    for (i64 w = threadIdx.x; w < m; w += 256) {
        const float p = row[w];
        s += (double)p;
        row[w] = sqrtf(fmaxf(p, 0.f));
    }
    red[threadIdx.x] = s;
    __syncthreads();
    for (int st = 128; st > 0; st >>= 1) {
        if ((int)threadIdx.x < st) red[threadIdx.x] += red[threadIdx.x + st];
        __syncthreads();
    }
    if (threadIdx.x == 0) l1[i] = red[0];
}

constexpr int HELL_TILE = 64;
constexpr int HELL_KSTEP = 32;
__global__ __launch_bounds__(256) void k_hell_gram(const float *__restrict__ R, int t, i64 m, i64 slice,
                                                   const int *__restrict__ tile_i, const int *__restrict__ tile_j,
                                                   double *__restrict__ partial ) {
    __shared__ float sa[HELL_KSTEP][HELL_TILE + 1], sb[HELL_KSTEP][HELL_TILE + 1];
    const int bi = tile_i[blockIdx.x] * HELL_TILE, bj = tile_j[blockIdx.x] * HELL_TILE;
    const i64 w0 = (i64)blockIdx.y * slice, w1 = min(m, w0 + slice);
    const int tx = threadIdx.x % 16, ty = threadIdx.x / 16;
    double acc[4][4];
    float facc[4][4];
#pragma unroll
    for (int a = 0; a < 4; ++a)
#pragma unroll
        for (int b = 0; b < 4; ++b) { acc[a][b] = 0.0; facc[a][b] = 0.f; }
    int since_flush = 0;
    for (i64 w = w0; w < w1; w += HELL_KSTEP) {
        for (int e = threadIdx.x; e < HELL_TILE * HELL_KSTEP; e += 256) {
            const int r = e / HELL_KSTEP, kk = e % HELL_KSTEP;
            const i64 ww = w + kk;
            sa[kk][r] = (bi + r < t && ww < w1) ? R[(i64)(bi + r) * m + ww] : 0.f;
            sb[kk][r] = (bj + r < t && ww < w1) ? R[(i64)(bj + r) * m + ww] : 0.f;
        }
        __syncthreads();
#pragma unroll 8
        for (int kk = 0; kk < HELL_KSTEP; ++kk) {
            float av[4], bv[4];
#pragma unroll
            for (int a = 0; a < 4; ++a) { av[a] = sa[kk][ty * 4 + a]; bv[a] = sb[kk][tx * 4 + a]; }
#pragma unroll
            for (int a = 0; a < 4; ++a)
#pragma unroll
                for (int b = 0; b < 4; ++b) facc[a][b] += av[a] * bv[b];
        }
        __syncthreads();
        since_flush += HELL_KSTEP;
        if (since_flush >= 256) {
#pragma unroll
            for (int a = 0; a < 4; ++a)
#pragma unroll
                for (int b = 0; b < 4; ++b) { acc[a][b] += (double)facc[a][b]; facc[a][b] = 0.f; }
            since_flush = 0;
        }
    }
    double *out = partial + (i64)blockIdx.y * t * t;
#pragma unroll
    for (int a = 0; a < 4; ++a)
#pragma unroll
        for (int b = 0; b < 4; ++b) {
            const int i = bi + ty * 4 + a, j = bj + tx * 4 + b;
            if (i < t && j < t) out[(i64)i * t + j] = acc[a][b] + (double)facc[a][b];
        }
}

__global__ __launch_bounds__(256) void k_hell_finish(const double *__restrict__ partial, int slices, int t,
                                                     const double *__restrict__ l1, double *__restrict__ D) {
    const i64 e = (i64)blockIdx.x * 256 + threadIdx.x;
    if (e >= (i64)t * t) return;
    const int i = (int)(e / t), j = (int)(e % t);
    const int a = min(i, j), b = max(i, j);
    double g = 0.0;
    for (int s = 0; s < slices; ++s) g += partial[(i64)s * t * t + (i64)a * t + b];
    const double li = l1[i], lj = l1[j];
    double d;
    if (i == j || (li == 0.0 && lj == 0.0)) d = 0.0;
    else if (li == 0.0 || lj == 0.0) d = 1.0;
    else d = sqrt(fmax(1.0 - g / sqrt(li * lj), 0.0));
    D[e] = d;
}

__device__ __forceinline__ float kl_log2(float p) {
    const bool tiny = p < 1.17549435e-38f;
    const float l = __log2f(tiny ? p * 4294967296.f : p);
    return tiny ? l - 32.f : l;
}

// ... 115 lines not shown
```

### enstop_amd/csrc/plsa_launch_plan.hpp

```cpp
#pragma once

#include <algorithm>
#include <cstdint>

namespace plsa {
namespace plan {

struct LaneShape { int kp, lpn, ch, row_lpn, row_ch; };
inline LaneShape lane_shape(int k, int chunks_per_lane, bool row_shape_8x2) {
    LaneShape s;
    s.kp = (k + 3) / 4 * 4;
    int lpn = 1;
    while (lpn < s.kp / 4 && lpn < 64) lpn *= 2;
    if (lpn >= 32 && lpn * 4 >= s.kp && chunks_per_lane == 2) lpn /= 2;
    s.lpn = lpn;
    s.ch = (s.kp / 4 + lpn - 1) / lpn;
    if (s.ch == 3) s.ch = 4;
    s.row_lpn = s.lpn; s.row_ch = s.ch;
    if (row_shape_8x2 && s.lpn == 16 && s.ch == 1 && s.kp == 64) { s.row_lpn = 8; s.row_ch = 2; }
    return s;
}

struct RowItems { bool use; int seg; };
inline RowItems row_items(int64_t n, int64_t nnz, int cus, int row_lpn, int ritems_mode, int rseg_override) {
    const int64_t group_slots = (int64_t)cus * 32 * (64 / std::max(1, row_lpn));
    const double avg = (double)nnz / (double)std::max<int64_t>(n, 1);
    const int rseg_decide = rseg_override ? rseg_override : 64;
    RowItems r;
    r.use = ritems_mode == 1 || (ritems_mode < 0 && n < 2 * group_slots && avg > 2.0 * rseg_decide);
    r.seg = rseg_override;
    if (!rseg_override) {
        const int64_t per_slot = nnz / std::max<int64_t>(group_slots, 1);
        r.seg = 16;
        while (r.seg * 2 <= per_slot && r.seg < 64) r.seg *= 2;
    }
    return r;
}

inline int col_item_len(int64_t nnz, int cus, int lpn, int seg_override) {
    const int64_t slots = (int64_t)cus * 32 * (64 / std::max(1, lpn));
    const int64_t want = nnz / std::max<int64_t>(slots + slots / 4, 1);
    int seg = 16;
    const int cap = 64;
    while (seg * 2 <= want && seg < cap) seg *= 2;
    return seg_override ? seg_override : seg;
}

inline int order_band(int kp, int order_band_knob) {
    const int band_bytes = (kp >= 64 ? 2048 : 512) << 10;
    return order_band_knob >= 0 ? order_band_knob : std::max(64, band_bytes / (kp > 0 ? kp * 4 : 256));
}

inline int sort_bits(int64_t count) {
    int bits = 1;
    while (((int64_t)1 << bits) < count) ++bits;
    return bits;
}

struct OrderKey { int len_bits, key_bits; };
inline OrderKey order_key(int64_t n, int band) {
    OrderKey k;
    k.len_bits = sort_bits(n + 1);
    k.key_bits = k.len_bits + (band > 0 ? sort_bits(n / band + 1) : 0);
    return k;
}

inline int e_item_len(int lpn, int eseg_override) {
    return eseg_override >= 0 ? eseg_override : (lpn >= 16 ? 64 : (lpn == 8 ? 8 : 16));
}

constexpr int64_t PACK_ID_RANGE = (int64_t)1 << 24;
inline bool packed_ok(int64_t nnz, int64_t id_range, uint64_t escaped) {
    return nnz > 0 && id_range <= PACK_ID_RANGE && escaped * 16 <= (uint64_t)nnz;
}

inline int grid_for(int64_t work, int per_block, int cap) {
    int64_t need = (work + per_block - 1) / per_block;
    if (need < 1) need = 1;
    return (int)std::min<int64_t>(need, cap);
}

struct RowPass { int grid, reduce_grid; };
inline RowPass row_pass(int64_t n, int64_t n_ritems, bool items, int row_lpn, int grid_cap, bool xcd_rows) {
    const int gpb = 256 / row_lpn;
    RowPass r;
    r.grid = grid_for(items ? n_ritems : n, gpb, grid_cap);
    if (xcd_rows) r.grid = (int)(((n + gpb - 1) / gpb + 7) / 8 * 8);
    r.reduce_grid = grid_for(n, gpb, grid_cap);
    return r;
}

struct ColPass { int n_chunks, reduce_grid, norm_blocks; };
inline ColPass col_pass(int64_t n_items, int64_t m, int lpn, int n_heavy, int grid_cap) {
    const int gpb = 256 / lpn;
    ColPass p;
    p.n_chunks = (int)((n_items + gpb - 1) / gpb);
    p.reduce_grid = grid_for(m, gpb, grid_cap) + n_heavy;
    p.norm_blocks = p.n_chunks > 2048 ? std::max(64, std::min(1024, p.n_chunks / 64)) : 0;
    return p;
}

inline bool xcd_split(bool xcd_split_knob, int n_chunks, int64_t n, int kp) {
    const bool u_fits_l2 = (double)n * kp * 4.0 <= 2.0 * 1024 * 1024;
    return xcd_split_knob && n_chunks >= 64 && !u_fits_l2;
}

inline void balance_lo(const double frac[9], int n_chunks, int lo[9]) {
    lo[0] = 0;
    for (int x = 1; x < 8; ++x) {
        const int v = (int)(frac[x] * n_chunks + 0.5);
        lo[x] = std::min(n_chunks, std::max(lo[x - 1], v));
    }
    lo[8] = n_chunks;
}

inline int col_grid(const int lo[9], int n_chunks, bool split) {
    int64_t g = n_chunks;
    if (split) {
        int longest = 1;
        for (int x = 0; x < 8; ++x) longest = std::max(longest, lo[x + 1] - lo[x]);
        g = 8 * (int64_t)longest;
    }
    return (int)std::max<int64_t>(1, std::min<int64_t>(g, (int64_t)1 << 22));
}

struct XcdTimes { double us[8], spread; };
inline XcdTimes xcd_times(const unsigned long long *stamps, int grid) {
    unsigned long long t0 = ~0ull, last[8] = {0, 0, 0, 0, 0, 0, 0, 0};
    for (int b = 0; b <= grid; ++b) if (stamps[b]) t0 = std::min(t0, stamps[b]);
    for (int b = 0; b < grid; ++b) last[b & 7] = std::max(last[b & 7], stamps[b]);
    XcdTimes t;
    double mean = 0.0, lo_t = 1e300, hi_t = 0.0;
    for (int x = 0; x < 8; ++x) {
        t.us[x] = std::max(1.0, (double)(last[x] - t0) / 100.0);
        mean += t.us[x] / 8.0; lo_t = std::min(lo_t, t.us[x]); hi_t = std::max(hi_t, t.us[x]);
    }
    t.spread = (hi_t - lo_t) / mean;
    return t;
}

inline void balance_step(const double frac[9], const double us[8], double next[9]) {
    double mean = 0.0, size[8], tot = 0.0;
    for (int x = 0; x < 8; ++x) mean += us[x] / 8.0;
    for (int x = 0; x < 8; ++x) {
        size[x] = std::max(1e-6, (frac[x + 1] - frac[x]) * (1.0 + 0.8 * (mean / us[x] - 1.0)));
        tot += size[x];
    }
    double acc = 0.0;
    next[0] = frac[0];
    for (int x = 0; x < 8; ++x) { acc += size[x]; next[x + 1] = acc / tot; }
    next[8] = 1.0;
}

inline bool table_is_wide(int64_t rows, int kp, bool force) { return force || (double)rows * kp * 4.0 >= 4294967296.0; }

}
}
```

### enstop_amd/csrc/plsa_member_kernels.hpp

```cpp
#pragma once

#include "plsa_kernels.hpp"

namespace plsa {

constexpr int MEMBERS_MAX = 64;

struct MemberArgs {
    const int4 *item_rec;
    const int *csc_row;
    const float *csc_val;
    float *partial;
    double *chunk_sums;
    i64 n_items;
    double *chunk_sums2;
    float *norm_pwz;
    const int *item_first, *heavy_cols;
    int n_chunks, norm_blocks;
    int m, n_heavy, heavy_items, reduce_grid;
    const int *indptr, *colidx;
    const float *vals;
    const int *row_order, *ritem_row, *ritem_start, *ritem_first;
    float *rpartial;
    double *ll_partials, *ll_out;
    i64 n_ritems;
    int n, rseg, row_grid, row_reduce_grid;
    float *U[2], *Vt[2];
};

__device__ __forceinline__ bool member_live(u64 live, unsigned r) { return (live >> r) & 1ull; }

template <class S, bool WANT_LL, bool TINY>
__global__ __launch_bounds__(256, PLSA_WAVES) void k_row_pass_members(const MemberArgs *__restrict__ args, u64 live, u64 cu,
                                                                      u64 cv, int kp_rt, float thresh) {
    const unsigned r = blockIdx.y;
    if (!member_live(live, r)) return;
    const MemberArgs &a = args[r];
    if (blockIdx.x >= (unsigned)a.row_grid) return;
    const int pu = (int)((cu >> r) & 1ull), pv = (int)((cv >> r) & 1ull);
    row_pass_body<S, false, WANT_LL, TINY>(a.indptr, a.colidx, a.vals, a.n, a.row_order, a.U[pu], a.Vt[pv], nullptr, a.U[1 - pu],
                                           nullptr, nullptr, kp_rt, thresh, a.ll_partials, a.ritem_row, a.ritem_start, a.rseg,
                                           a.n_ritems, a.rpartial, 0, blockIdx.x, (unsigned)a.row_grid);
}

template <class S>
__global__ __launch_bounds__(256) void k_row_reduce_members(const MemberArgs *__restrict__ args, u64 live, u64 cu, int kp_rt) {
    const unsigned r = blockIdx.y;
    if (!member_live(live, r)) return;
    const MemberArgs &a = args[r];
    if (!a.ritem_row || blockIdx.x >= (unsigned)a.row_reduce_grid) return;
    const int pu = (int)((cu >> r) & 1ull);
    row_reduce_body<S>(a.ritem_first, a.n, a.rpartial, a.U[1 - pu], nullptr, kp_rt, blockIdx.x, (unsigned)a.row_reduce_grid);
}

__global__ __launch_bounds__(256) void k_ll_final_members(const MemberArgs *__restrict__ args, u64 live) {
    __shared__ double red[256];
    const unsigned r = blockIdx.x;
    if (!member_live(live, r)) return;
    const MemberArgs &a = args[r];
    ll_final_body(a.ll_partials, a.row_grid, a.ll_out, red);
}

template <class S, bool TINY>
__global__ __launch_bounds__(256, PLSA_WAVES_COL) void k_col_pass_members(const MemberArgs *__restrict__ args, u64 live, u64 cu,
                                                                          u64 cv, int kp_rt, float thresh) {
    extern __shared__ double scol[];
    const unsigned r = blockIdx.y;
    if (!member_live(live, r)) return;
    const MemberArgs &a = args[r];
    if (blockIdx.x >= (unsigned)a.n_chunks) return;
    const int pu = (int)((cu >> r) & 1ull), pv = (int)((cv >> r) & 1ull);
    const unsigned nblocks = min((unsigned)a.n_chunks, gridDim.x);
    col_pass_body<S, false, false, TINY>(a.item_rec, a.n_items, nullptr, a.csc_row, a.csc_val, nullptr, a.U[pu], a.Vt[pv], nullptr,
                                         nullptr, a.partial, kp_rt, thresh, 0, a.chunk_sums, nullptr, scol, blockIdx.x, nblocks);
}

__global__ __launch_bounds__(256) void k_norm_reduce_members(const MemberArgs *__restrict__ args, u64 live, int kp) {
    __shared__ double sred[256];
    const unsigned r = blockIdx.y;
    if (!member_live(live, r)) return;
    const MemberArgs &a = args[r];
    if (blockIdx.x >= (unsigned)a.norm_blocks) return;
    norm_reduce_body(a.chunk_sums, a.n_chunks, kp, a.chunk_sums2, sred, blockIdx.x, (unsigned)a.norm_blocks);
}

__global__ __launch_bounds__(256) void k_colsum_final_members(const MemberArgs *__restrict__ args, u64 live, int kp) {
    __shared__ double sred[256];
    const unsigned r = blockIdx.x;
    if (!member_live(live, r)) return;
    const MemberArgs &a = args[r];
    if (a.norm_blocks > 0) colsum_final_body(a.chunk_sums2, a.norm_blocks, kp, a.norm_pwz, sred);
    else colsum_final_body(a.chunk_sums, a.n_chunks, kp, a.norm_pwz, sred);
}

template <class S>
__global__ __launch_bounds__(256) void k_col_reduce_norm_members(const MemberArgs *__restrict__ args, u64 live, u64 cv,
                                                                 int kp_rt) {
    extern __shared__ float sdyn[];
    const unsigned r = blockIdx.y;
    if (!member_live(live, r)) return;
    const MemberArgs &a = args[r];
    if (blockIdx.x >= (unsigned)a.reduce_grid) return;
    const int kp = S::kp(kp_rt);
    constexpr int GPB = 256 / S::LPN;
    float *snorm = sdyn + GPB * kp;
    for (int z = threadIdx.x; z < kp; z += 256) snorm[z] = a.norm_pwz[z];
    __syncthreads();
    const int pv = (int)((cv >> r) & 1ull);
    col_reduce_body<S, true>(a.item_first, a.m, a.heavy_items, a.heavy_cols, a.n_heavy, a.partial, a.Vt[1 - pv], kp,
                             (int)blockIdx.x, a.reduce_grid, sdyn, snorm);
}

}
```

### enstop_amd/csrc/plsa_members.hpp

```cpp
#pragma once

struct plsa_members {
    struct MemberDelete {
        void operator()(plsa_ctx *m) const {
            if (!m) return;
            m->stream.h = nullptr; m->stream2.h = nullptr;
            delete m;
        }
    };
    using Member = std::unique_ptr<plsa_ctx, MemberDelete>;
    plsa_ctx *leader = nullptr;
    std::vector<Member> ctx;
    std::vector<char> prepared;
    struct Info { int group = -1, group_size = 0, items = 0, rseg = 0, n_chunks = 0, n_heavy = 0, row_grid = 0, norm_blocks = 0; };
    std::vector<Info> info;
    std::vector<double> last_ll;
    DevBuf table, ll_out;
    Pinned<double> h_ll;
};

namespace {

int new_member(plsa_ctx *leader, plsa_members::Member &out) {
    plsa_members::Member m(new plsa_ctx());
    m->device = leader->device;
    m->prop = leader->prop;
    m->stream.h = leader->stream.h;
    m->stream2.h = leader->stream2.h;
    m->ls = m->stream;
    if (hipEventCreateWithFlags(&m->ev_fork.h, hipEventDisableTiming) != hipSuccess ||
        hipEventCreateWithFlags(&m->ev_join.h, hipEventDisableTiming) != hipSuccess ||
        hipEventCreateWithFlags(&m->ev_row.h, hipEventDisableTiming) != hipSuccess ||
        hipEventCreateWithFlags(&m->ev_tail.h, hipEventDisableTiming) != hipSuccess ||
        hipEventCreateWithFlags(&m->ev_ll.h, hipEventDisableTiming) != hipSuccess ||
        host_alloc(m->h_ll, 2) != hipSuccess)
        return fail(leader, "plsa_members: event / pinned buffer creation failed");
    read_knobs(m.get());
    out = std::move(m);
    return 0;
}

struct ScratchLoan {
    plsa_ctx *l, *m;
    void swap_all() {
        for (auto p : {&plsa_ctx::tmp0, &plsa_ctx::tmp1, &plsa_ctx::tmp2, &plsa_ctx::cubtmp, &plsa_ctx::pk_count, &plsa_ctx::mt_words,
                       &plsa_ctx::mt_state, &plsa_ctx::mt_fin, &plsa_ctx::mt_poly, &plsa_ctx::mt_seq})
            (l->*p).swap(m->*p);
    }
    ScratchLoan(plsa_ctx *l_, plsa_ctx *m_) : l(l_), m(m_) { swap_all(); }
    ~ScratchLoan() { swap_all(); }
};

int member_rc(plsa_ctx *leader, plsa_ctx *m, int rc) {
    if (rc) leader->err = m->err;
    return rc;
}

int members_check(plsa_members *b, int32_t member) {
    if (!b) return fail(nullptr, "plsa_members: NULL batch");
    if (member < 0 || member >= (int32_t)b->ctx.size())
        return fail(b->leader, "plsa_members: member %d outside [0, %d)", member, (int)b->ctx.size());
    return 0;
}

int member_args(plsa_ctx *c, double *ll_out, plsa::MemberArgs &a, plsa_members::Info &inf) {
    ColLaunch l;
    RowLaunch r;
    CHK(prepare_col_pass(c, false, l));
    CHK(prepare_row_pass(c, false, true, r));
    a = plsa::MemberArgs{};
    a.item_rec = l.item_rec;
    a.csc_row = l.csc_row;
    a.csc_val = l.csc_val;
    a.partial = l.partial;
    a.chunk_sums = l.colsum_rows;
    a.n_items = l.n_items;
    a.chunk_sums2 = l.colsum_rows2;
    a.norm_pwz = l.norm_pwz;
    a.item_first = l.item_first;
    a.heavy_cols = l.heavy_cols;
    a.n_chunks = l.plan.n_chunks;
    a.norm_blocks = l.plan.norm_blocks;
    a.m = (int)c->m;
    a.n_heavy = l.n_heavy;
    a.heavy_items = l.heavy_items;
    a.reduce_grid = l.plan.reduce_grid;
    a.indptr = r.indptr;
    a.colidx = r.colidx;
    a.vals = r.vals;
    a.row_order = r.order;
    a.ritem_row = r.ritem_row;
    a.ritem_start = r.ritem_start;
    a.ritem_first = r.ritem_first;
    a.rpartial = r.rpartial;
    a.ll_partials = r.ll_partials;
    a.ll_out = ll_out;
    a.n_ritems = r.n_ritems;
    a.n = (int)c->n;
    a.rseg = r.rseg;
    a.row_grid = r.plan.grid;
    a.row_reduce_grid = r.plan.reduce_grid;
    for (int i = 0; i < 2; ++i) { a.U[i] = c->U[i].as<float>(); a.Vt[i] = c->Vt[i].as<float>(); }
    inf.items = r.items; inf.rseg = r.rseg; inf.n_chunks = l.plan.n_chunks; inf.n_heavy = l.n_heavy;
    inf.row_grid = r.plan.grid; inf.norm_blocks = l.plan.norm_blocks;
    return 0;
}

template <class Fn>
int dispatch_narrow_row(plsa_ctx *c, Fn &&fn) {
    if (c->row_lpn == 8 && c->row_ch == 2 && c->kp == 64) { fn(plsa::Shape<8, 2, true>{}); return 0; }
    return dispatch_shape(c, fn);
}

int fit_group(plsa_members *b, const std::vector<int> &who, const std::vector<plsa::MemberArgs> &rows, int n_iter,
              int n_iter_per_test, double tolerance, float thresh, int flags, int32_t *iters_done, float *ll_trace, int ll_cap,
              int32_t *n_ll) {
    plsa_ctx *L = b->leader, *c0 = b->ctx[who[0]].get();
    const int G = (int)who.size();
    const bool trace = flags & PLSA_TRACE_LL;
    HIPCHK(L, hipMemcpyAsync(b->table.p, rows.data(), sizeof(plsa::MemberArgs) * (size_t)G, hipMemcpyHostToDevice, L->stream));
    HIPCHK(L, hipStreamSynchronize(L->stream));
    const plsa::MemberArgs *table = b->table.as<plsa::MemberArgs>();
    int row_x = 1, reduce_x = 1, chunks_x = 1, norm_x = 0, rr_x = 0;
    for (const auto &a : rows) {
        row_x = std::max(row_x, a.row_grid);
        reduce_x = std::max(reduce_x, a.reduce_grid);
        chunks_x = std::max(chunks_x, a.n_chunks);
        norm_x = std::max(norm_x, a.norm_blocks);
        if (a.ritem_row) rr_x = std::max(rr_x, a.row_reduce_grid);
    }
    const bool pk_row = c0->packed && c0->pk_csr.ok, pk_col = c0->packed && c0->pk_csc.ok;
    const bool tiny = thresh < plsa::TINY_THRESH;
    const int kp = c0->kp;
    using u64 = unsigned long long;
    u64 live = G == 64 ? ~0ull : ((1ull << G) - 1ull), cu = 0, cv = 0;
    for (int g = 0; g < G; ++g) {
        plsa_ctx *c = b->ctx[who[g]].get();
        if (c->cu) cu |= 1ull << g;
        if (c->cv) cv |= 1ull << g;
    }
    using F = std::false_type;
    const bool two_streams = L->overlap;
    hipStream_t col_stream = two_streams ? L->stream2.h : L->stream.h;
    auto row_pass = [&](bool want_ll) -> int {
        CHK(dispatch_narrow_row(c0, [&](auto S) {
            using Sh = decltype(S);
            select_row_pass<Sh>(pk_row, F{}, want_ll, tiny, [&](auto SS, auto, auto LL, auto TN) {
                hipLaunchKernelGGL((plsa::k_row_pass_members<decltype(SS), decltype(LL)::value, decltype(TN)::value>),
                                   dim3(row_x, G), dim3(256), 0, L->stream, table, live, cu, cv, kp, thresh);
            });
            if (rr_x > 0)
                hipLaunchKernelGGL((plsa::k_row_reduce_members<Sh>), dim3(rr_x, G), dim3(256), 0, L->stream, table, live, cu, kp);
        }));
        if (want_ll) {
            hipLaunchKernelGGL(plsa::k_ll_final_members, dim3(G), dim3(256), 0, L->stream, table, live);
            HIPCHK(L, hipMemcpyAsync(b->h_ll.get(), b->ll_out.p, sizeof(double) * (size_t)G, hipMemcpyDeviceToHost, L->stream));
        }
        return launch_check(L, "k_row_pass_members");
    };
    auto col_chain = [&]() -> int {
        CHK(dispatch_shape(c0, [&](auto S) {
            using Sh = decltype(S);
            constexpr int GPB = 256 / Sh::LPN;
            const size_t smem = sizeof(double) * (size_t)GPB * kp;
            select_col_pass<Sh>(pk_col, F{}, F{}, tiny, [&](auto SS, auto, auto, auto TN) {
                hipLaunchKernelGGL((plsa::k_col_pass_members<decltype(SS), decltype(TN)::value>), dim3(chunks_x, G), dim3(256),
                                   smem, col_stream, table, live, cu, cv, kp, thresh);
            });
            if (norm_x > 0)
                hipLaunchKernelGGL(plsa::k_norm_reduce_members, dim3(norm_x, G), dim3(256), 0, col_stream, table, live, kp);
            hipLaunchKernelGGL(plsa::k_colsum_final_members, dim3(G), dim3(256), 0, col_stream, table, live, kp);
            hipLaunchKernelGGL((plsa::k_col_reduce_norm_members<Sh>), dim3(reduce_x, G), dim3(256),
                               sizeof(float) * (size_t)(GPB + 1) * kp, col_stream, table, live, cv, kp);
        }));
        return launch_check(L, "k_col_pass_members");
    };
    std::vector<plsa::fit::Tests> tests;
    for (int g = 0; g < G; ++g)
        tests.push_back({ll_trace ? ll_trace + (size_t)who[g] * ll_cap : nullptr, tolerance,
                         (flags & PLSA_STOP_NO_ZERO_ARM) ? plsa::fit::FIT_NO_ZERO_ARM : plsa::fit::FIT, n_iter_per_test, ll_cap});
    std::vector<int> iters(G, 0);
    bool pending = false, first = true;
    for (int i = 0; i < n_iter && live; ++i) {
        const bool want_ll = pending || first;
        if (two_streams) {
            HIPCHK(L, hipEventRecord(L->ev_fork, L->stream));
            HIPCHK(L, hipStreamWaitEvent(L->stream2, L->ev_fork, 0));
        }
        CHK(col_chain());
        if (two_streams) HIPCHK(L, hipEventRecord(L->ev_join, L->stream2));
        CHK(row_pass(want_ll));
        if (two_streams) HIPCHK(L, hipStreamWaitEvent(L->stream, L->ev_join, 0));
        if (want_ll) {
            HIPCHK(L, hipStreamSynchronize(L->stream));
            for (int g = 0; g < G; ++g) {
                if (!((live >> g) & 1ull)) continue;
                b->last_ll[who[g]] = b->h_ll[g];
                if (first) tests[g].initial(b->h_ll[g]);
                else if (tests[g].test(b->h_ll[g])) live &= ~(1ull << g);
            }
            first = false;
        }
        cu ^= live; cv ^= live;
        for (int g = 0; g < G; ++g) if ((live >> g) & 1ull) iters[g]++;
        pending = tests[0].due_after(i);
    }
    HIPCHK(L, hipStreamSynchronize(L->stream));
    for (int g = 0; g < G; ++g) {
        plsa_ctx *c = b->ctx[who[g]].get();
        c->cu = (int)((cu >> g) & 1ull); c->cv = (int)((cv >> g) & 1ull);
        c->p_state.invalidate();
        if (((live >> g) & 1ull) && pending && trace) {
            ScratchLoan loan(L, c);
            double ll = 0.0;
            CHK(member_rc(L, c, run_loglik(c, nullptr, &ll)));
            b->last_ll[who[g]] = ll;
            tests[g].trailing(ll);
        }
        iters_done[who[g]] = iters[g];
        n_ll[who[g]] = tests[g].count;
    }
    return 0;
}

}

extern "C" {

int plsa_members_create(plsa_ctx *ctx, int32_t n_members, plsa_members **out) {
    if (!out) return fail(ctx, "plsa_members_create: out is NULL");
    *out = nullptr;
    if (!ctx) return fail(nullptr, "plsa_members_create: NULL context");
    if (n_members < 1 || n_members > PLSA_MEMBERS_MAX)
        return fail(ctx, "plsa_members_create: n_members=%d outside [1, %d]", n_members, (int)PLSA_MEMBERS_MAX);
    static_assert(PLSA_MEMBERS_MAX == plsa::MEMBERS_MAX, "the live mask is one 64-bit word");
    HIPCHK(ctx, hipSetDevice(ctx->device));
    std::unique_ptr<plsa_members> b(new plsa_members());
    b->leader = ctx;
    b->ctx.resize(n_members);
    b->prepared.assign(n_members, 0);
    b->info.assign(n_members, plsa_members::Info{});
    b->last_ll.assign(n_members, 0.0);
// ... 161 lines not shown
```

### enstop_amd/csrc/plsa_nmf.hpp

```cpp
#pragma once

namespace {

int nmf_ready(plsa_ctx *c, const char *who) {
    HIPCHK(c, hipSetDevice(c->device));
    if (c->n <= 0) return fail(c, "%s: no corpus uploaded", who);
    if (c->k <= 0 || !c->U[0].p || !c->Vt[0].p) return fail(c, "%s: factors not set (call plsa_nmf_set_factors)", who);
    if (c->k > 1024) return fail(c, "%s: k=%d outside [1,1024]", who, c->k);
    return need_factors(c);
}

int nmf_factor_sum(plsa_ctx *c, int which) {
    const i64 rows = which ? c->m : c->n;
    const float *A = which ? c->Vt[c->cv].as<float>() : c->U[c->cu].as<float>();
    const int nb = (int)std::min<i64>(plsa::NORM_BLOCKS, std::max<i64>(1, rows));
    CHK(ensure(c, c->nmf.slabs, sizeof(double) * (size_t)plsa::NORM_BLOCKS * c->kp));
    CHK(ensure(c, c->nmf.raw, sizeof(double) * 2 * (size_t)c->kp));
    CHK(ensure(c, c->nmf.guarded, sizeof(float) * 2 * (size_t)c->kp));
    {
        Scope s(c, "k_nmf_colsum_partial");
        hipLaunchKernelGGL(plsa::k_nmf_colsum_partial, dim3(nb), dim3(256), 0, c->ls, A, rows, c->kp, c->nmf.slabs.as<double>());
    }
    {
        Scope s(c, "k_nmf_colsum_final");
        hipLaunchKernelGGL(plsa::k_nmf_colsum_final, dim3(1), dim3(256), 0, c->ls, c->nmf.slabs.as<double>(), nb, c->kp,
                           c->nmf.raw.as<double>() + (size_t)which * c->kp, c->nmf.guarded.as<float>() + (size_t)which * c->kp,
                           which ? plsa::NMF_EPS32 : 1.0f);
    }
    return launch_check(c, "k_nmf_colsum");
}

bool nmf_row_items(plsa_ctx *c) { return c->ritems.use && c->ritems.n > 0; }

int nmf_run_update_w(plsa_ctx *c, int iters) {
    RowLaunch r;
    CHK(prepare_row_pass(c, false, false, r));
    if (r.items && iters != 1) return fail(c, "internal: the combined NMF pass needs whole documents");
    c->p_state.invalidate();
    CHK(dispatch_shape_row(c, [&](auto S) {
        using Sh = decltype(S);
        const float *Vt = c->Vt[c->cv].as<float>(), *hs = c->nmf.guarded.as<float>() + c->kp;
        float *W = c->U[c->cu].as<float>();
        const int n = (int)c->n, kp = c->kp;
        auto launch = [&](auto SS) {
            Scope s(c, "k_nmf_row_pass");
            hipLaunchKernelGGL((plsa::k_nmf_row_pass<decltype(SS)>), dim3(r.plan.grid), dim3(256), 0, c->ls, r.indptr, r.colidx,
                               r.vals, n, r.order, W, Vt, hs, kp, iters, r.ritem_row, r.ritem_start, r.rseg, r.n_ritems, r.rpartial);
        };
        if (r.packed) launch(plsa::Packed<Sh>{}); else launch(Sh{});
        if (r.items) {
            Scope s(c, "k_nmf_row_reduce");
            hipLaunchKernelGGL((plsa::k_nmf_row_reduce<Sh>), dim3(r.plan.reduce_grid), dim3(256), 0, c->ls,
                               r.ritem_first, n, r.rpartial, W, hs, kp);
        }
    }));
    return launch_check(c, "k_nmf_row_pass");
}

int nmf_run_update_h(plsa_ctx *c) {
    ColLaunch l;
    CHK(prepare_col_pass(c, false, l));
    CHK(nmf_factor_sum(c, 0));
    c->p_state.invalidate();
    CHK(dispatch_shape_gather(c, table_is_wide(c, c->n), [&](auto S) {
        using Sh = decltype(S);
        const int grid = plsa::plan::col_grid(nullptr, l.plan.n_chunks, false);
        const float *W = c->U[c->cu].as<float>(), *Vt = c->Vt[c->cv].as<float>();
        auto launch = [&](auto SS) {
            Scope s(c, "k_nmf_col_pass");
            hipLaunchKernelGGL((plsa::k_nmf_col_pass<decltype(SS)>), dim3(grid), dim3(256), 0, c->ls, l.item_rec, l.n_items,
                               l.csc_row, l.csc_val, W, Vt, l.partial, c->kp);
        };
        if (l.packed) launch(plsa::Packed<Sh>{}); else launch(Sh{});
    }));
    CHK(launch_check(c, "k_nmf_col_pass"));
    CHK(run_col_pass(c, false, nullptr, 0.f, 2));
    {
        Scope s(c, "k_nmf_h_finish");
        const i64 total4 = c->m * c->kp / 4;
        hipLaunchKernelGGL(plsa::k_nmf_h_finish, dim3(grid_for(c, total4, 256)), dim3(256), c->kp * sizeof(float), c->ls,
                           c->Vacc.as<float>(), c->Vt[c->cv].as<float>(), c->m, c->kp, c->nmf.guarded.as<float>());
    }
    return launch_check(c, "k_nmf_h_finish");
}

int nmf_run_divergence(plsa_ctx *c, double *out) {
    CHK(nmf_factor_sum(c, 0));
    CHK(nmf_factor_sum(c, 1));
    RowLaunch r;
    CHK(prepare_row_pass(c, true, false, r));
    const int grid = r.plan.reduce_grid;
    const int *order = r.order;
    if (r.items) CHK(ensure_roworder(c, &order));
    CHK(ensure(c, c->nmf.obj, sizeof(double) * 2 * (size_t)grid));
    CHK(ensure(c, c->nmf.out, sizeof(double) * 2));
    CHK(dispatch_shape_row(c, [&](auto S) {
        Scope s(c, "k_nmf_divergence");
        hipLaunchKernelGGL((plsa::k_nmf_divergence<decltype(S)>), dim3(grid), dim3(256), 0, c->ls, r.indptr, r.colidx, r.vals,
                           (int)c->n, order, c->U[c->cu].as<float>(), c->Vt[c->cv].as<float>(), c->kp, c->nmf.obj.as<double>());
    }));
    {
        Scope s(c, "k_nmf_divergence_final");
        hipLaunchKernelGGL(plsa::k_nmf_divergence_final, dim3(1), dim3(256), 0, c->ls, c->nmf.obj.as<double>(), grid,
                           c->nmf.raw.as<double>(), c->nmf.raw.as<double>() + c->kp, c->k, c->nmf.out.as<double>());
    }
    CHK(launch_check(c, "k_nmf_divergence"));
    double h[2] = {0.0, 0.0};
    HIPCHK(c, hipMemcpyAsync(h, c->nmf.out.p, sizeof h, hipMemcpyDeviceToHost, c->ls));
    HIPCHK(c, hipStreamSynchronize(c->ls));
    *out = h[0];
    return 0;
}

}

extern "C" {

int plsa_nmf_set_factors(plsa_ctx *c, const float *W, const float *H, int64_t n, int64_t m, int32_t k) {
    if (!W || !H) return fail(c, "plsa_nmf_set_factors: W and H must both be given");
    return plsa_set_factors(c, W, H, n, m, k);
}

int plsa_nmf_get_factors(plsa_ctx *c, float *W, float *H) {
    CHK(nmf_ready(c, "plsa_nmf_get_factors"));
    return plsa_get_factors(c, W, H);
}

int plsa_nmf_update_w(plsa_ctx *c) {
    CHK(nmf_ready(c, "plsa_nmf_update_w"));
    CHK(nmf_factor_sum(c, 1));
    CHK(nmf_run_update_w(c, 1));
    HIPCHK(c, hipStreamSynchronize(c->ls));
    return 0;
}

int plsa_nmf_update_h(plsa_ctx *c) {
    CHK(nmf_ready(c, "plsa_nmf_update_h"));
    CHK(nmf_run_update_h(c));
    HIPCHK(c, hipStreamSynchronize(c->ls));
    return 0;
}

int plsa_nmf_divergence(plsa_ctx *c, double *sqrt2d) {
    CHK(nmf_ready(c, "plsa_nmf_divergence"));
    if (!sqrt2d) return fail(c, "plsa_nmf_divergence: NULL argument");
    return nmf_run_divergence(c, sqrt2d);
}

int plsa_nmf_fit(plsa_ctx *c, int update_h, int max_iter, double tol, int32_t *n_iter, double *errors, int32_t errors_len) {
    CHK(nmf_ready(c, "plsa_nmf_fit"));
    if (max_iter < 1) return fail(c, "plsa_nmf_fit: max_iter=%d, expected at least 1", max_iter);
    int n_err = 0;
    auto record = [&](double e) { if (errors && n_err < errors_len) errors[n_err] = e; n_err++; };
    double error_at_init = 0.0;
    CHK(nmf_run_divergence(c, &error_at_init));
    record(error_at_init);
    double previous = error_at_init;
    CHK(ensure_ritems(c));
    const bool combined = !update_h && !nmf_row_items(c);
    if (!update_h) CHK(nmf_factor_sum(c, 1));
    int it = 0;
    while (it < max_iter) {
        if (combined) {
            const int next = tol > 0 ? std::min(max_iter, (it / 10 + 1) * 10) : max_iter;
            CHK(nmf_run_update_w(c, next - it));
            it = next;
        } else {
            if (update_h) CHK(nmf_factor_sum(c, 1));
            CHK(nmf_run_update_w(c, 1));
            if (update_h) CHK(nmf_run_update_h(c));
            it++;
        }
        if (tol > 0 && it % 10 == 0) {
            double error = 0.0;
            CHK(nmf_run_divergence(c, &error));
            record(error);
            if ((previous - error) / error_at_init < tol) break;
            previous = error;
        }
    }
    HIPCHK(c, hipStreamSynchronize(c->ls));
    if (n_iter) *n_iter = it;
    return 0;
}

}
```

### enstop_amd/csrc/plsa_nmf_kernels.hpp

```cpp
#pragma once

#include "plsa_kernels.hpp"

namespace plsa {

constexpr float NMF_EPS32 = 1.1920928955078125e-07f;
constexpr float NMF_EPS64 = 2.220446049250313e-16f;

template <int CH>
__device__ __forceinline__ float nmf_dot(const float4 (&a)[CH], const float4 (&b)[CH]) {
#pragma clang fp contract(off)
    float p = 0.f;
#pragma unroll
    for (int j = 0; j < CH; ++j) {
        p = __builtin_fmaf(a[j].x, b[j].x, p); p = __builtin_fmaf(a[j].y, b[j].y, p);
        p = __builtin_fmaf(a[j].z, b[j].z, p); p = __builtin_fmaf(a[j].w, b[j].w, p);
    }
    return p;
}

template <int CH>
__device__ __forceinline__ void nmf_axpy(float4 (&acc)[CH], float q, const float4 (&r)[CH]) {
#pragma clang fp contract(off)
#pragma unroll
    for (int j = 0; j < CH; ++j) {
        acc[j].x = __builtin_fmaf(q, r[j].x, acc[j].x); acc[j].y = __builtin_fmaf(q, r[j].y, acc[j].y);
        acc[j].z = __builtin_fmaf(q, r[j].z, acc[j].z); acc[j].w = __builtin_fmaf(q, r[j].w, acc[j].w);
    }
}

__device__ __forceinline__ float nmf_quotient(float x, float wh) {
#pragma clang fp contract(off)
    return x / (wh < NMF_EPS32 ? NMF_EPS32 : wh);
}

__device__ __forceinline__ float4 nmf_scale(const float4 &f, const float4 &num, const float4 &den) {
#pragma clang fp contract(off)
    return make_float4(f.x * (num.x / den.x), f.y * (num.y / den.y), f.z * (num.z / den.z), f.w * (num.w / den.w));
}

template <class S, int UN>
__device__ __forceinline__ void nmf_batch(int s0, int id_l, float x_l, int li, int kp, const float *table,
                                          const float4 (&own)[S::CH], float4 (&acc)[S::CH]) {
    constexpr int LPN = S::LPN, CH = S::CH;
    float4 a[UN][CH];
#pragma unroll
    for (int q = 0; q < UN; ++q) gather_row<S>(table, __shfl(id_l, s0 + q, LPN), li, kp, a[q]);
    float mine = 1.f;
#pragma unroll
    for (int q = 0; q < UN; ++q) {
        const float wh = group_sum<LPN>(nmf_dot<CH>(own, a[q]));
        mine = (li == s0 + q) ? wh : mine;
    }
    const float q_mine = nmf_quotient(x_l, mine);
#pragma unroll
    for (int q = 0; q < UN; ++q) nmf_axpy<CH>(acc, __shfl(q_mine, s0 + q, LPN), a[q]);
}

template <class S, int UN>
__device__ __forceinline__ void nmf_sweep(const int *__restrict__ ids, const float *__restrict__ vals, int j0, int j1,
                                          int li, int kp, const float *table, const float4 (&own)[S::CH],
                                          float4 (&acc)[S::CH]) {
    constexpr int LPN = S::LPN;
    int id_n = (j0 + li < j1) ? ldi(ids + j0 + li) : 0;
    float x_n = (!S::PACKED && j0 + li < j1) ? ldf(vals + j0 + li) : 0.f;
    for (int jb = j0; jb < j1; jb += LPN) {
        int id_l = id_n;
        float x_l = x_n;
        if (S::PACKED) unpack_entry(id_l, x_l, vals, jb + li, j1);
        const int jn = jb + LPN + li;
        id_n = jn < j1 ? ldi(ids + jn) : 0;
        if (!S::PACKED) x_n = jn < j1 ? ldf(vals + jn) : 0.f;
        const int cnt = min(LPN, j1 - jb);
        int s0 = 0;
        for (; s0 + UN <= cnt; s0 += UN) nmf_batch<S, UN>(s0, id_l, x_l, li, kp, table, own, acc);
        constexpr int TAIL = (UN >= 2 && LPN >= 2) ? 2 : 1;
        for (; s0 < cnt; s0 += TAIL) nmf_batch<S, TAIL>(s0, id_l, x_l, li, kp, table, own, acc);
    }
}

template <class S>
__global__ __launch_bounds__(256) void k_nmf_row_pass(const int *__restrict__ indptr, const int *__restrict__ colidx,
                                                      const float *__restrict__ vals, int n,
                                                      const int *__restrict__ row_order, float *W,
                                                      const float *__restrict__ Vt, const float *__restrict__ h_sum,
                                                      int kp_rt, int iters, const int *__restrict__ ritem_row,
                                                      const int *__restrict__ ritem_start, int rseg, i64 n_ritems,
                                                      float *__restrict__ rpartial) {
    constexpr int LPN = S::LPN, CH = S::CH;
    constexpr int GPB = 256 / LPN;
    const int kp = S::kp(kp_rt);
    const int li = threadIdx.x % LPN;
    const int gid = threadIdx.x / LPN;
    const bool items = ritem_row != nullptr;
    const i64 n_work = items ? n_ritems : (i64)n;
    float4 hs[CH];
    load_row<S, false>(h_sum, li, kp, hs);
    for (i64 r = (i64)blockIdx.x * GPB + gid; r < n_work; r += (i64)gridDim.x * GPB) {
        const int d = items ? ritem_row[r] : (row_order ? row_order[r] : (int)r);
        const int j0 = items ? ritem_start[r] : indptr[d];
        const int j1 = items ? min(j0 + rseg, indptr[d + 1]) : indptr[d + 1];
        float4 w[CH], acc[CH];
        load_row<S, true>(W + (i64)d * kp, li, kp, w);
        for (int it = 0; it < iters; ++it) {
#pragma unroll
            for (int j = 0; j < CH; ++j) acc[j] = zero4();
            nmf_sweep<S, S::UNR>(colidx, vals, j0, j1, li, kp, Vt, w, acc);
            if (items) break;
#pragma unroll
            for (int j = 0; j < CH; ++j) w[j] = S::ok(li, j, kp) ? nmf_scale(w[j], acc[j], hs[j]) : zero4();
        }
#pragma unroll
        for (int j = 0; j < CH; ++j) {
            if (!S::ok(li, j, kp)) continue;
            if (items) st4(rpartial + r * kp + S::c4(li, j), acc[j]);
            else st4(W + (i64)d * kp + S::c4(li, j), w[j]);
        }
    }
}

template <class S>
__global__ __launch_bounds__(256) void k_nmf_row_reduce(const int *__restrict__ ritem_first, int n,
                                                        const float *__restrict__ rpartial, float *W,
                                                        const float *__restrict__ h_sum, int kp_rt) {
    constexpr int LPN = S::LPN, CH = S::CH;
    constexpr int GPB = 256 / LPN;
    const int kp = S::kp(kp_rt);
    const int li = threadIdx.x % LPN;
    const int gid = threadIdx.x / LPN;
    float4 hs[CH];
    load_row<S, false>(h_sum, li, kp, hs);
    for (i64 d = (i64)blockIdx.x * GPB + gid; d < n; d += (i64)gridDim.x * GPB) {
        const int i0 = ritem_first[d], i1 = ritem_first[d + 1];
        float4 acc[CH], w[CH];
#pragma unroll
        for (int j = 0; j < CH; ++j) acc[j] = zero4();
        for (int it = i0; it < i1; ++it) {
            float4 p[CH];
            load_row<S, true>(rpartial + (i64)it * kp, li, kp, p);
#pragma unroll
            for (int j = 0; j < CH; ++j) {
                acc[j].x += p[j].x; acc[j].y += p[j].y; acc[j].z += p[j].z; acc[j].w += p[j].w;
            }
        }
        load_row<S, true>(W + d * kp, li, kp, w);
#pragma unroll
        for (int j = 0; j < CH; ++j)
            if (S::ok(li, j, kp)) st4(W + d * kp + S::c4(li, j), nmf_scale(w[j], acc[j], hs[j]));
    }
}

template <class S>
__global__ __launch_bounds__(256) void k_nmf_col_pass(const int4 *__restrict__ item_rec, i64 n_items,
                                                      const int *__restrict__ csc_row, const float *__restrict__ csc_val,
                                                      const float *__restrict__ W, const float *__restrict__ Vt,
                                                      float *__restrict__ partial, int kp_rt) {
    constexpr int LPN = S::LPN, CH = S::CH;
    constexpr int GPB = 256 / LPN;
    const int kp = S::kp(kp_rt);
    const int li = threadIdx.x % LPN;
    const int gid = threadIdx.x / LPN;
    for (i64 io = (i64)blockIdx.x * GPB + gid; io < n_items; io += (i64)gridDim.x * GPB) {
        const int4 rec = item_rec[io];
        float4 h[CH], acc[CH];
        load_row<S, true>(Vt + (i64)rec.x * kp, li, kp, h);
#pragma unroll
        for (int j = 0; j < CH; ++j) acc[j] = zero4();
        nmf_sweep<S, S::UNR_COL>(csc_row, csc_val, rec.y, rec.z, li, kp, W, h, acc);
#pragma unroll
        for (int j = 0; j < CH; ++j)
            if (S::ok(li, j, kp)) st4(partial + (i64)rec.w * kp + S::c4(li, j), acc[j]);
    }
}

__global__ __launch_bounds__(256) void k_nmf_h_finish(const float *__restrict__ num, float *Vt, i64 m, int kp,
                                                      const float *__restrict__ w_sum) {
    extern __shared__ float s_wsum[];
    for (int z = threadIdx.x; z < kp; z += 256) s_wsum[z] = w_sum[z];
    __syncthreads();
    const i64 total4 = m * kp / 4;
    const int kq = kp / 4;
    for (i64 i = (i64)blockIdx.x * 256 + threadIdx.x; i < total4; i += (i64)gridDim.x * 256) {
        const int z4 = (int)(i % kq) * 4;
        float4 o = nmf_scale(ld4(Vt + i * 4), ld4(num + i * 4), make_float4(s_wsum[z4], s_wsum[z4 + 1], s_wsum[z4 + 2], s_wsum[z4 + 3]));
        o.x = o.x < NMF_EPS64 ? 0.f : o.x; o.y = o.y < NMF_EPS64 ? 0.f : o.y;
        o.z = o.z < NMF_EPS64 ? 0.f : o.z; o.w = o.w < NMF_EPS64 ? 0.f : o.w;
        st4(Vt + i * 4, o);
    }
}

__global__ __launch_bounds__(256) void k_nmf_colsum_partial(const float *__restrict__ A, i64 rows, int kp,
                                                            double *__restrict__ partials) {
    __shared__ double sred[256];
    const i64 per = (rows + gridDim.x - 1) / gridDim.x;
    const i64 r0 = (i64)blockIdx.x * per, r1 = min(rows, r0 + per);
    for (int zb = 0; zb < kp; zb += 256) {
        const int span = min(256, kp - zb);
        const int rpp = 256 / span;
        const int z = zb + (int)threadIdx.x % span;
        const int ro = (int)threadIdx.x / span;
        double s = 0.0;
        if (ro < rpp)
            for (i64 r = r0 + ro; r < r1; r += rpp) s += (double)A[r * kp + z];
        sred[threadIdx.x] = (ro < rpp) ? s : 0.0;
        __syncthreads();
        if ((int)threadIdx.x < span) {
            double tot = 0.0;
            for (int r = 0; r < rpp; ++r) tot += sred[r * span + threadIdx.x];
            partials[(i64)blockIdx.x * kp + zb + threadIdx.x] = tot;
        }
        __syncthreads();
    }
}

__global__ __launch_bounds__(256) void k_nmf_colsum_final(const double *__restrict__ partials, int n_partials, int kp,
                                                          double *__restrict__ raw, float *__restrict__ guarded,
                                                          float if_zero) {
    for (int z = threadIdx.x; z < kp; z += 256) {
        double t = 0.0;
        for (int b = 0; b < n_partials; ++b) t += partials[(i64)b * kp + z];
        raw[z] = t;
        const float f = (float)t;
        guarded[z] = f == 0.f ? if_zero : f;
    }
}

template <class S>
__global__ __launch_bounds__(256) void k_nmf_divergence(const int *__restrict__ indptr, const int *__restrict__ colidx,
                                                        const float *__restrict__ vals, int n,
                                                        const int *__restrict__ row_order, const float *__restrict__ W,
                                                        const float *__restrict__ Vt, int kp_rt,
                                                        double *__restrict__ partials ) {
    constexpr int LPN = S::LPN, CH = S::CH, UNR = S::UNR;
    constexpr int GPB = 256 / LPN;
    const int kp = S::kp(kp_rt);
    const int li = threadIdx.x % LPN;
    const int gid = threadIdx.x / LPN;
    double s_log = 0.0, s_x = 0.0;
    for (i64 r = (i64)blockIdx.x * GPB + gid; r < n; r += (i64)gridDim.x * GPB) {
        const int d = row_order ? row_order[r] : (int)r;
        const int j0 = indptr[d], j1 = indptr[d + 1];
        float4 w[CH];
        load_row<S, true>(W + (i64)d * kp, li, kp, w);
        for (int jb = j0; jb < j1; jb += LPN) {
            const bool mine_ok = jb + li < j1;
            const int id_l = mine_ok ? ldi(colidx + jb + li) : 0;
            const float x_l = mine_ok ? ldf(vals + jb + li) : 0.f;
            const int cnt = min(LPN, j1 - jb);
            float mine = 1.f;
            for (int s0 = 0; s0 < cnt; s0 += UNR) {
                float4 a[UNR][CH];
#pragma unroll
                for (int q = 0; q < UNR; ++q) gather_row<S>(Vt, __shfl(id_l, s0 + q, LPN), li, kp, a[q]);
#pragma unroll
                for (int q = 0; q < UNR; ++q) {
                    const float wh = group_sum<LPN>(nmf_dot<CH>(w, a[q]));
                    mine = (li == s0 + q) ? wh : mine;
                }
            }
            if (mine_ok && x_l > NMF_EPS32) {
                const double wh = (double)(mine < NMF_EPS32 ? NMF_EPS32 : mine);
                s_log += (double)x_l * log((double)x_l / wh);
                s_x += (double)x_l;
            }
        }
    }
    __shared__ double red[256];
    for (int which = 0; which < 2; ++which) {
        red[threadIdx.x] = which ? s_x : s_log;
        __syncthreads();
        for (int s = 128; s > 0; s >>= 1) {
            if ((int)threadIdx.x < s) red[threadIdx.x] += red[threadIdx.x + s];
            __syncthreads();
        }
        if (threadIdx.x == 0) partials[(i64)which * gridDim.x + blockIdx.x] = red[0];
        __syncthreads();
    }
}

__global__ __launch_bounds__(256) void k_nmf_divergence_final(const double *__restrict__ partials, int nb,
                                                              const double *__restrict__ w_sum_raw,
                                                              const double *__restrict__ h_sum_raw, int k,
                                                              double *__restrict__ out ) {
    __shared__ double red[256];
    __shared__ double sums[2];
    for (int which = 0; which < 2; ++which) {
        ll_final_body(partials + (i64)which * nb, nb, sums + which, red);
        __syncthreads();
    }
    if (threadIdx.x == 0) {
        double wh = 0.0;
        for (int z = 0; z < k; ++z) wh += w_sum_raw[z] * h_sum_raw[z];
        const double D = sums[0] + (wh - sums[1]);
        out[0] = sqrt(2.0 * (D > 0.0 ? D : 0.0));
        out[1] = D;
    }
}

}
```

### enstop_amd/csrc/plsa_structures.hpp

```cpp
#pragma once

namespace {

static_assert(plsa::plan::PACK_ID_RANGE == plsa::PACK_MAX_IDS, "the packing rule and the packed word disagree on the id bits");

void set_active_pointers(plsa_ctx *c) {
    if (c->active_is_base) {
        c->indptr = c->b_indptr.as<int>(); c->col = c->b_col.as<int>(); c->val = c->b_val.as<float>();
        c->n = c->bn; c->m = c->bm; c->nnz = c->bnnz;
    } else {
        c->indptr = c->a_indptr.as<int>(); c->col = c->a_col.as<int>(); c->val = c->a_val.as<float>();
    }
    c->rowidx.invalidate(); c->csc.invalidate(); c->pk_csr.invalidate(); c->pk_csc.invalidate(); c->roworder.invalidate();
    c->ritems.invalidate(); c->eitems.invalidate(); c->p_state.invalidate(); c->ref_heavy.invalidate(); c->ref_tsum.invalidate();
    c->ref_blocks.invalidate();
    c->ref_pairs_off = false;
}

void set_shape(plsa_ctx *c, int k) {
    const plsa::plan::LaneShape sh = plsa::plan::lane_shape(k, c->chunks_per_lane, c->row_shape_8x2);
    const int prev_lpn = c->struct_lpn, prev_row_lpn = c->struct_row_lpn, lpn = sh.lpn;
    c->k = k; c->kp = sh.kp;
    c->lpn = sh.lpn; c->ch = sh.ch;
    c->row_lpn = sh.row_lpn; c->row_ch = sh.row_ch;
    if (c->row_lpn != prev_row_lpn) {
        c->ritems.invalidate();
        c->struct_row_lpn = c->row_lpn;
    }
    if (lpn != prev_lpn) {
        c->eitems.invalidate();
        if (!c->seg_override) { c->csc.invalidate(); c->pk_csc.invalidate(); }
        c->struct_lpn = lpn;
    }
}

template <class Call>
int cub_two_phase(plsa_ctx *c, const char *what, Call &&call) {
    size_t bytes = 0;
    hipError_t e = call(nullptr, bytes);
    if (e == hipSuccess) {
        CHK(ensure(c, c->cubtmp, bytes));
        e = call(c->cubtmp.p, bytes);
    }
    return e == hipSuccess ? 0 : fail(c, "%s failed: %s", what, hipGetErrorString(e));
}

int exclusive_sum_int(plsa_ctx *c, const int *in, int *out, i64 count) {
    auto scan = [&](void *tmp, size_t &bytes) {
        return hipcub::DeviceScan::ExclusiveSum(tmp, bytes, in, out, (int)count, c->stream);
    };
    return cub_two_phase(c, "hipcub::DeviceScan::ExclusiveSum", scan);
}

int ensure_rowidx(plsa_ctx *c) {
    if (c->rowidx.valid) return 0;
    CHK(ensure(c, c->rowidx.ids, sizeof(int) * (size_t)c->nnz));
    if (c->n > 0) {
        Scope s(c, "k_expand_rows");
        hipLaunchKernelGGL(plsa::k_expand_rows, dim3(grid_for(c, c->n, 4)), dim3(256), 0, c->stream,
                           c->indptr, (int)c->n, c->rowidx.ids.as<int>());
    }
    CHK(launch_check(c, "k_expand_rows"));
    c->rowidx.valid = true;
    return 0;
}

int row_xcd_range(const plsa_ctx *c) {
    const i64 gpb = 256 / std::max(1, c->row_lpn);
    if (!c->row_xcd || c->n < 64 * gpb) return 0;
    return (int)(((c->n + gpb - 1) / gpb + 7) / 8 * gpb);
}

int ensure_roworder(plsa_ctx *c, const int **out) {
    *out = nullptr;
    if (!c->sort_rows) return 0;
    const int range = row_xcd_range(c);
    if (!c->roworder.valid || c->roworder.range != range) {
        c->roworder.range = range;
        const i64 n = c->n;
        CHK(ensure(c, c->roworder.ids, sizeof(int) * (size_t)n));
        CHK(ensure(c, c->tmp0, sizeof(int) * (size_t)n * 2));
        CHK(ensure(c, c->tmp1, sizeof(int) * (size_t)n));
        int *len = c->tmp0.as<int>(), *len_sorted = c->tmp0.as<int>() + n, *ids = c->tmp1.as<int>();
        hipLaunchKernelGGL(plsa::k_row_lengths, dim3((unsigned)((n + 255) / 256)), dim3(256), 0, c->stream,
                           c->indptr, (int)n, len, ids, range);
        CHK(launch_check(c, "k_row_lengths"));
        auto sort = [&](void *tmp, size_t &bytes) {
            return hipcub::DeviceRadixSort::SortPairsDescending(tmp, bytes, len, len_sorted, ids, c->roworder.ids.as<int>(), (int)n,
                                                                0, 32, c->stream);
        };
        CHK(cub_two_phase(c, "hipcub::DeviceRadixSort::SortPairsDescending", sort));
        c->roworder.valid = true;
    }
    *out = c->roworder.ids.as<int>();
    return 0;
}

template <class Fill>
int cut_items(plsa_ctx *c, const int *ptr, i64 count, int seg, DevBuf &first, std::initializer_list<DevBuf *> arrays, i64 *n_items,
              Fill &&fill) {
    CHK(ensure(c, first, sizeof(int) * (size_t)(count + 1)));
    CHK(ensure(c, c->tmp0, sizeof(int) * (size_t)(count + 1)));
    HIPCHK(c, hipMemsetAsync(c->tmp0.p, 0, sizeof(int) * (size_t)(count + 1), c->stream));
    hipLaunchKernelGGL(plsa::k_item_counts, dim3((unsigned)((count + 255) / 256)), dim3(256), 0, c->stream,
                       ptr, (int)count, seg, c->tmp0.as<int>());
    CHK(exclusive_sum_int(c, c->tmp0.as<int>(), first.as<int>(), count + 1));
    int cnt = 0;
    HIPCHK(c, hipMemcpyAsync(&cnt, first.as<int>() + count, sizeof(int), hipMemcpyDeviceToHost, c->stream));
    HIPCHK(c, hipStreamSynchronize(c->stream));
    *n_items = cnt;
    for (DevBuf *a : arrays) CHK(ensure(c, *a, sizeof(int) * (size_t)std::max(cnt, 1)));
    return fill(cnt);
}

int fill_row_items(plsa_ctx *c, const DevBuf &first, int seg, DevBuf &row, DevBuf &start) {
    hipLaunchKernelGGL(plsa::k_ritem_fill, dim3((unsigned)((c->n + 255) / 256)), dim3(256), 0, c->stream,
                       c->indptr, first.as<int>(), (int)c->n, seg, row.as<int>(), start.as<int>());
    return launch_check(c, "k_ritem_fill");
}

int ensure_ritems(plsa_ctx *c) {
    if (c->ritems.valid) return 0;
    plsa_ctx::RowItems &r = c->ritems;
    const plsa::plan::RowItems ri = plsa::plan::row_items(c->n, c->nnz, c->prop.multiProcessorCount, c->row_lpn, c->ritems_mode,
                                                          c->rseg_override);
    r.use = ri.use;
    r.seg = ri.seg;
    r.n = 0;
    if (r.use)
        CHK(cut_items(c, c->indptr, c->n, r.seg, r.first, {&r.row, &r.start}, &r.n,
                      [&](int) { return fill_row_items(c, r.first, r.seg, r.row, r.start); }));
    r.valid = true;
    return 0;
}

int ensure_eitems(plsa_ctx *c, int eseg) {
    plsa_ctx::EItems &e = c->eitems;
    if (e.valid && e.seg == eseg) return 0;
    e.seg = eseg;
    e.n = 0;
    if (eseg > 0) {
        CHK(cut_items(c, c->indptr, c->n, eseg, c->tmp1, {&e.row, &e.start}, &e.n,
                      [&](int) { return fill_row_items(c, c->tmp1, eseg, e.row, e.start); }));
        HIPCHK(c, hipStreamSynchronize(c->stream));
    }
    e.valid = true;
    return 0;
}

int packed_begin(plsa_ctx *c, plsa_ctx::PackedStream &s, i64 id_range, bool *pack) {
    s.invalidate();
    s.ok = false;
    *pack = c->packed && plsa::plan::packed_ok(c->nnz, id_range, 0);
    if (!*pack) return 0;
    CHK(ensure(c, s.buf, sizeof(unsigned) * (size_t)c->nnz));
    CHK(ensure(c, c->pk_count, sizeof(unsigned long long)));
    HIPCHK(c, hipMemsetAsync(c->pk_count.p, 0, sizeof(unsigned long long), c->stream));
    return 0;
}

int packed_finish(plsa_ctx *c, plsa_ctx::PackedStream &s, i64 id_range, bool pack) {
    unsigned long long escaped = 0;
    if (pack) {
        HIPCHK(c, hipMemcpyAsync(&escaped, c->pk_count.p, sizeof escaped, hipMemcpyDeviceToHost, c->stream));
        HIPCHK(c, hipStreamSynchronize(c->stream));
    }
    s.ok = pack && plsa::plan::packed_ok(c->nnz, id_range, escaped);
    if (!s.ok) s.buf.release();
    s.valid = true;
    return 0;
}

int build_packed(plsa_ctx *c, plsa_ctx::PackedStream &s, const int *ids, const float *vals, i64 id_range) {
    bool pack = false;
    CHK(packed_begin(c, s, id_range, &pack));
    if (pack) {
        hipLaunchKernelGGL(plsa::k_pack_entries, dim3(grid_for(c, c->nnz, 256)), dim3(256), 0, c->stream,
                           ids, vals, c->nnz, s.buf.as<unsigned>(), c->pk_count.as<unsigned long long>());
        CHK(launch_check(c, "k_pack_entries"));
    }
    return packed_finish(c, s, id_range, pack);
}

int csc_order_entries(plsa_ctx *c, bool pack) {
    plsa_ctx::Csc &s = c->csc;
    const i64 nnz = c->nnz, m = c->m;
    if (nnz <= 0) {
        HIPCHK(c, hipMemsetAsync(s.colptr.p, 0, sizeof(int) * (size_t)(m + 1), c->stream));
        return 0;
    }
    hipLaunchKernelGGL(plsa::k_iota, dim3(grid_for(c, nnz, 256)), dim3(256), 0, c->stream, c->tmp1.as<int>(), nnz);
    const int bits = plsa::plan::sort_bits(m);
    auto sort = [&](void *tmp, size_t &bytes) {
        return hipcub::DeviceRadixSort::SortPairs(tmp, bytes, c->col, c->tmp0.as<int>(), c->tmp1.as<int>(), s.pos.as<int>(), nnz, 0,
                                                  bits, c->stream);
    };
    CHK(cub_two_phase(c, "hipcub::DeviceRadixSort::SortPairs", sort));
    hipLaunchKernelGGL(plsa::k_colptr_from_sorted, dim3((unsigned)((m + 256) / 256)), dim3(256), 0, c->stream,
                       c->tmp0.as<int>(), nnz, (int)m, s.colptr.as<int>());
    hipLaunchKernelGGL(plsa::k_csc_gather, dim3(grid_for(c, nnz, 256)), dim3(256), 0, c->stream,
                       s.pos.as<int>(), c->rowidx.ids.as<int>(), c->val, nnz, s.row.as<int>(), s.val.as<float>(),
                       pack ? c->pk_csc.buf.as<unsigned>() : nullptr, pack ? c->pk_count.as<unsigned long long>() : nullptr);
    return launch_check(c, "k_csc_gather");
}

int csc_items_in_visiting_order(plsa_ctx *c) {
    plsa_ctx::Csc &s = c->csc;
    const int band = plsa::plan::order_band(c->kp, c->order_band);
    const plsa::plan::OrderKey key = plsa::plan::order_key(c->n, band);
    CHK(cut_items(c, s.colptr.as<int>(), c->m, s.seg, s.item_first, {&s.item_col, &s.item_start, &s.item_end, &s.item_order},
                  &s.n_items, [&](int n_items) {
        const size_t ni = (size_t)std::max(n_items, 1);
        CHK(ensure(c, c->tmp2, sizeof(unsigned long long) * ni * 2));
        CHK(ensure(c, c->tmp1, sizeof(int) * ni));
        if (n_items > 0)
            hipLaunchKernelGGL(plsa::k_item_fill, dim3((unsigned)((n_items + 255) / 256)), dim3(256), 0, c->stream,
                               s.colptr.as<int>(), s.item_first.as<int>(), (int)c->m, s.seg, s.row.as<int>(), s.item_col.as<int>(),
                               s.item_start.as<int>(), s.item_end.as<int>(), band, key.len_bits, c->tmp2.as<unsigned long long>(),
                               c->tmp1.as<int>(), n_items);
        return launch_check(c, "k_item_fill");
    }));
    if (s.n_items > 0) {
        unsigned long long *d_key = c->tmp2.as<unsigned long long>();
        auto sort = [&](void *tmp, size_t &bytes) {
            return hipcub::DeviceRadixSort::SortPairs(tmp, bytes, d_key, d_key + s.n_items, c->tmp1.as<int>(), s.item_order.as<int>(),
                                                      (int)s.n_items, 0, key.key_bits, c->stream);
        };
        CHK(cub_two_phase(c, "hipcub::DeviceRadixSort::SortPairs", sort));
    }
    return 0;
}

int csc_item_records(plsa_ctx *c) {
    plsa_ctx::Csc &s = c->csc;
    CHK(ensure(c, s.item_rec, sizeof(int4) * (size_t)std::max<i64>(s.n_items, 1)));
    if (s.n_items > 0) {
        hipLaunchKernelGGL(plsa::k_item_records, dim3((unsigned)((s.n_items + 255) / 256)), dim3(256), 0, c->stream,
                           c->use_item_order ? s.item_order.as<int>() : nullptr, s.item_col.as<int>(),
                           s.item_start.as<int>(), s.item_end.as<int>(), s.n_items, s.item_rec.as<int4>());
        CHK(launch_check(c, "k_item_records"));
    }
    s.balanced = false;
    return 0;
}

int csc_heavy_list(plsa_ctx *c) {
    plsa_ctx::Csc &s = c->csc;
    const i64 m = c->m;
    CHK(ensure(c, s.heavy_cols, sizeof(int) * (size_t)(m + 1)));
    HIPCHK(c, hipMemsetAsync(s.heavy_cols.as<int>() + m, 0, sizeof(int), c->stream));
    hipLaunchKernelGGL(plsa::k_heavy_list, dim3((unsigned)((m + 255) / 256)), dim3(256), 0, c->stream,
                       s.item_first.as<int>(), (int)m, c->heavy_items, s.heavy_cols.as<int>(), s.heavy_cols.as<int>() + m);
    CHK(launch_check(c, "k_heavy_list"));
    HIPCHK(c, hipMemcpyAsync(&s.n_heavy, s.heavy_cols.as<int>() + m, sizeof(int), hipMemcpyDeviceToHost, c->stream));
    return 0;
}

int ensure_csc(plsa_ctx *c) {
    if (c->csc.valid) return 0;
    CHK(ensure_rowidx(c));
    c->csc.seg = plsa::plan::col_item_len(c->nnz, c->prop.multiProcessorCount, c->lpn, c->seg_override);
    const i64 nnz = c->nnz, m = c->m;
    CHK(ensure(c, c->csc.colptr, sizeof(int) * (size_t)(m + 1)));
    CHK(ensure(c, c->csc.row, sizeof(int) * (size_t)nnz));
    CHK(ensure(c, c->csc.val, sizeof(float) * (size_t)nnz));
    CHK(ensure(c, c->csc.pos, sizeof(int) * (size_t)nnz));
    CHK(ensure(c, c->tmp0, sizeof(int) * (size_t)std::max<i64>(nnz, m + 1)));
    CHK(ensure(c, c->tmp1, sizeof(int) * (size_t)nnz));
    bool pack = false;
    CHK(packed_begin(c, c->pk_csc, c->n, &pack));
    CHK(csc_order_entries(c, pack));
    CHK(csc_items_in_visiting_order(c));
    CHK(csc_item_records(c));
    CHK(csc_heavy_list(c));
    if (!pack) HIPCHK(c, hipStreamSynchronize(c->stream));
    CHK(packed_finish(c, c->pk_csc, c->n, pack));
    c->csc.valid = true;
    return 0;
}

int ensure_packed_csr(plsa_ctx *c) {
    if (!c->packed || c->pk_csr.valid) return 0;
    return build_packed(c, c->pk_csr, c->col, c->val, c->m);
}

int ensure_packed_csc(plsa_ctx *c) {
    CHK(ensure_csc(c));
    if (!c->packed || c->pk_csc.valid) return 0;
    return build_packed(c, c->pk_csc, c->csc.row.as<int>(), c->csc.val.as<float>(), c->n);
}

int balance_set_lo(plsa_ctx *c, int n_chunks) {
    plsa::plan::balance_lo(c->bal_frac, n_chunks, c->bal_lo);
    c->bal_chunks = n_chunks;
    HIPCHK(c, hipMemcpyAsync(c->csc.xcd_lo.p, c->bal_lo, sizeof(int) * 9, hipMemcpyHostToDevice, c->ls));
    return 0;
}

template <class Launch>
int ensure_balance(plsa_ctx *c, int n_chunks, bool split, Launch &&launch) {
    if (c->csc.balanced && c->bal_chunks == n_chunks) return 0;
    CHK(ensure(c, c->csc.xcd_lo, sizeof(int) * 16));
    const bool warm = c->bal_have_frac;
    if (!warm) for (int x = 0; x <= 8; ++x) c->bal_frac[x] = x / 8.0;
    CHK(balance_set_lo(c, n_chunks));
    c->bal_launches = 0;
    const bool small_grid_active = c->small_grid > 0 && (double)c->nnz * c->kp < c->overlap_full_limit;
    const bool tune = split && n_chunks >= 64 && !small_grid_active &&
                      (c->balance > 0 || (c->balance < 0 && (double)c->nnz * c->kp >= 1e8));
    if (tune) {
        const size_t cap = (size_t)8 * (size_t)n_chunks + 16;
        CHK(ensure(c, c->t_end, sizeof(unsigned long long) * cap));
        std::vector<unsigned long long> te;
        const int max_launches = warm ? 1 : 8;
        if (!warm) CHK(launch(false));
        double best_spread = 1e300, best_frac[9];
        std::copy(c->bal_frac, c->bal_frac + 9, best_frac);
        for (int it = 0; it < max_launches; ++it) {
            const int grid = plsa::plan::col_grid(c->bal_lo, n_chunks, split);
            te.assign((size_t)grid + 1, 0);
            HIPCHK(c, hipMemsetAsync(c->t_end.p, 0, sizeof(unsigned long long) * ((size_t)grid + 1), c->ls));
            CHK(launch(true));
            HIPCHK(c, hipMemcpyAsync(te.data(), c->t_end.p, sizeof(unsigned long long) * ((size_t)grid + 1),
                                     hipMemcpyDeviceToHost, c->ls));
            HIPCHK(c, hipStreamSynchronize(c->ls));
            c->bal_launches++;
            const plsa::plan::XcdTimes t = plsa::plan::xcd_times(te.data(), grid);
            std::copy(t.us, t.us + 8, c->bal_end_us);
            if (t.spread < best_spread) {
                best_spread = t.spread;
                std::copy(c->bal_frac, c->bal_frac + 9, best_frac);
            }
            if (t.spread <= 0.02) break;
            const bool out_of_launches = it == max_launches - 1 && !warm;
            if (out_of_launches) std::copy(best_frac, best_frac + 9, c->bal_frac);
            else plsa::plan::balance_step(c->bal_frac, t.us, c->bal_frac);
            CHK(balance_set_lo(c, n_chunks));
            if (out_of_launches) break;
        }
        c->bal_have_frac = true;
    }
    c->csc.balanced = true;
    return 0;
}

}
```

Baseline: 345.9 iter/s.

## Lay out packed entry streams in lane-interleaved blocks for 16-byte loads

Packed CSR and CSC entry streams are rewritten into padded per-row/per-item blocks where each lane's four consecutive entries sit contiguously, so the row and column passes can fetch four packed entries with one int4 (optionally nontemporal) load instead of a scalar load per entry. A new EntryCursor abstracts the prefetch, and the pack kernel now maps output words back to source entries through block/item tables. This adds padding memory, a binary search in the packing kernel, and new rebuild/invalidation logic when lane counts or segment sizes change.

Measured after the change: 365.5 iter/s (median of 6 runs). 1.06x the previous value.

```diff
diff --git a/enstop_amd/csrc/plsa_hip.hip b/enstop_amd/csrc/plsa_hip.hip
--- a/enstop_amd/csrc/plsa_hip.hip
+++ b/enstop_amd/csrc/plsa_hip.hip
@@ -131,7 +131,11 @@
     bool packed = true;
     struct PackedStream : Derived<PackedStream> {
         DevBuf buf;
+        DevBuf blk;
+        int lpn = 0, seg = 0;
+        i64 words = 0;
         bool ok = false;
+        bool reshape = false;
         int state() const { return !valid ? -1 : (ok ? 1 : 0); }
     } pk_csr, pk_csc;
     DevBuf pk_count;
@@ -705,6 +709,7 @@
     bool items, packed, xcd_rows;
     const int *indptr, *colidx;
     const float *vals;
+    const int *sblk;
     const int *order;
     const int *ritem_row, *ritem_start, *ritem_first;
     float *rpartial;
@@ -725,6 +730,7 @@
     if (!from_p) CHK(ensure_packed_csr(c));
     r.packed = !from_p && c->packed && c->pk_csr.ok;
     r.indptr = c->indptr; r.colidx = r.packed ? c->pk_csr.buf.as<int>() : c->col; r.vals = c->val;
+    r.sblk = r.packed && !r.items ? c->pk_csr.blk.as<int>() : nullptr;
     r.ritem_row = r.items ? c->ritems.row.as<int>() : nullptr;
     r.ritem_start = r.items ? c->ritems.start.as<int>() : nullptr;
     r.ritem_first = r.items ? c->ritems.first.as<int>() : nullptr;
@@ -746,7 +752,8 @@
         select_row_pass<Sh>(r.packed, from_p, want_ll, thresh < plsa::TINY_THRESH, [&](auto SS, auto FP, auto LL, auto TN) {
             Scope s(c, from_p ? "k_row_pass<P>" : want_ll ? "k_row_pass<fused,LL>" : "k_row_pass<fused>");
             hipLaunchKernelGGL((plsa::k_row_pass<decltype(SS), decltype(FP)::value, decltype(LL)::value, decltype(TN)::value>),
-                               dim3(r.plan.grid), dim3(256), 0, c->ls, r.indptr, r.colidx, r.vals, n, r.order, U, Vt, p_base(c), Un,
+                               dim3(r.plan.grid), dim3(256), 0, c->ls, r.indptr, r.colidx, r.vals, r.sblk, n, r.order, U, Vt, p_base(c),
+                               Un,
                                d_sw, d_norm_pdz, kp, thresh, r.ll_partials, r.ritem_row, r.ritem_start, r.rseg, r.n_ritems,
                                r.rpartial, r.xcd_rows ? 1 : 0);
         });
@@ -769,6 +776,7 @@
     i64 n_items;
     const int *csc_row, *csc_pos;
     const float *csc_val;
+    int slot;
     float *partial;
     double *colsum_rows, *colsum_rows2;
     float *norm_pwz;
@@ -788,6 +796,7 @@
     l.item_rec = c->csc.item_rec.as<int4>(); l.n_items = c->csc.n_items;
     l.csc_row = l.packed ? c->pk_csc.buf.as<int>() : c->csc.row.as<int>();
     l.csc_pos = c->csc.pos.as<int>(); l.csc_val = c->csc.val.as<float>();
+    l.slot = l.packed ? plsa::plan::line_slot(c->pk_csc.seg, c->pk_csc.lpn) : 0;
     l.partial = c->partial.as<float>(); l.norm_pwz = c->norm_pwz.as<float>();
     l.colsum_rows = c->colsum_rows.as<double>(); l.colsum_rows2 = c->colsum_rows2.as<double>();
     l.item_first = c->csc.item_first.as<int>(); l.heavy_cols = c->csc.heavy_cols.as<int>();
@@ -816,7 +825,8 @@
                 unsigned long long *te = c->t_end.as<unsigned long long>();
                 select_col_pass<Sh>(l.packed, from_p, timed, thresh < plsa::TINY_THRESH, [&](auto SS, auto FP, auto TM, auto TN) {
                     hipLaunchKernelGGL((plsa::k_col_pass<decltype(SS), decltype(FP)::value, decltype(TM)::value, decltype(TN)::value>),
-                                       dim3(grid), dim3(256), smem, c->ls, l.item_rec, l.n_items, lo, l.csc_row, l.csc_val, l.csc_pos,
+                                       dim3(grid), dim3(256), smem, c->ls, l.item_rec, l.n_items, lo, l.csc_row, l.csc_val, l.slot,
+                                       l.csc_pos,
                                        U, Vt, p_base(c), d_sw, l.partial, kp, thresh, l.xcd_split, l.colsum_rows, te);
                 });
                 return launch_check(c, "k_col_pass");
diff --git a/enstop_amd/csrc/plsa_kernels.hpp b/enstop_amd/csrc/plsa_kernels.hpp
--- a/enstop_amd/csrc/plsa_kernels.hpp
+++ b/enstop_amd/csrc/plsa_kernels.hpp
@@ -1,6 +1,8 @@
 #pragma once
 #include <hip/hip_runtime.h>
 #include <stdint.h>
+
+#include "plsa_launch_plan.hpp"
 
 #ifndef PLSA_UNR
 #define PLSA_UNR 4
@@ -93,6 +95,50 @@
     x = (float)(e >> 24);
     if (x == 0.f && j < j_end) x = ldf(vals + j);
 }
+
+template <int LPN>
+__device__ __forceinline__ int row_item_slot(int rseg) { return (rseg + 4 * LPN - 1) / (4 * LPN) * (4 * LPN); }
+
+template <class S>
+struct EntryCursor {
+    static constexpr int LPN = S::LPN;
+    int4 cur;
+    float x_n;
+    int soff, c;
+
+    __device__ __forceinline__ static int4 ld_block(const int *p) {
+        typedef int i4v __attribute__((ext_vector_type(4)));
+        const i4v *q = reinterpret_cast<const i4v *>(p);
+        const i4v t = PLSA_NT_STREAMS ? __builtin_nontemporal_load(q) : *q;
+        return make_int4(t.x, t.y, t.z, t.w);
+    }
+    __device__ __forceinline__ void open(const int *__restrict__ ids, const float *__restrict__ vals, int sbase, int j0, int j1,
+                                         int li) {
+        if constexpr (S::PACKED) {
+            soff = sbase - j0 + 4 * li;
+            c = 0;
+            cur = j0 < j1 ? ld_block(ids + soff + j0) : make_int4(0, 0, 0, 0);
+        } else {
+            cur.x = (j0 + li < j1) ? ldi(ids + j0 + li) : 0;
+            x_n = (j0 + li < j1) ? ldf(vals + j0 + li) : 0.f;
+        }
+    }
+    __device__ __forceinline__ void take(const int *__restrict__ ids, const float *__restrict__ vals, int jb, int j1, int li,
+                                         int &id_l, float &x_l) {
+        if constexpr (S::PACKED) {
+            id_l = c == 0 ? cur.x : c == 1 ? cur.y : c == 2 ? cur.z : cur.w;
+            unpack_entry(id_l, x_l, vals, jb + li, j1);
+            if (c == 3) cur = (jb + LPN < j1) ? ld_block(ids + soff + jb + LPN) : make_int4(0, 0, 0, 0);
+            c = (c + 1) & 3;
+        } else {
+            id_l = cur.x;
+            x_l = x_n;
+            const int jn = jb + LPN + li;
+            cur.x = jn < j1 ? ldi(ids + jn) : 0;
+            x_n = jn < j1 ? ldf(vals + jn) : 0.f;
+        }
+    }
+};
 
 template <class S, bool ZERO_INVALID, bool STREAM = false>
 __device__ __forceinline__ void load_row(const float *row, int li, int kp, float4 (&out)[S::CH]) {
@@ -272,7 +318,7 @@
 template <class S, bool FROM_P, bool WANT_LL, bool TINY>
 __device__ __forceinline__ void row_pass_body(const int *__restrict__ indptr,
                                                   const int *__restrict__ colidx,
-                                                  const float *__restrict__ vals, int n,
+                                                  const float *__restrict__ vals, const int *__restrict__ sblk, int n,
                                                   const int *__restrict__ row_order,
                                                   const float *__restrict__ U,
                                                   const float *__restrict__ Vt,
@@ -303,15 +349,12 @@
 #pragma unroll
         for (int j = 0; j < CH; ++j) acc[j] = zero4();
         const float swd = (WANT_LL && sw) ? sw[d] : 1.0f;
-        int w_n = (j0 + li < j1) ? ldi(colidx + j0 + li) : 0;
-        float x_n = (!S::PACKED && j0 + li < j1) ? ldf(vals + j0 + li) : 0.f;
+        EntryCursor<S> es;
+        es.open(colidx, vals, S::PACKED ? (items ? (int)r * row_item_slot<LPN>(rseg) : sblk[d] * (4 * LPN)) : 0, j0, j1, li);
         for (int jb = j0; jb < j1; jb += LPN) {
-            int w_l = w_n;
-            float x_l = x_n;
-            if (S::PACKED) unpack_entry(w_l, x_l, vals, jb + li, j1);
-            const int jn = jb + LPN + li;
-            w_n = jn < j1 ? ldi(colidx + jn) : 0;
-            if (!S::PACKED) x_n = jn < j1 ? ldf(vals + jn) : 0.f;
+            int w_l;
+            float x_l;
+            es.take(colidx, vals, jb, j1, li, w_l, x_l);
             const int cnt = min(LPN, j1 - jb);
             for (int s0 = 0; s0 < cnt; s0 += UNR) {
                 float4 a[UNR][CH];
@@ -412,7 +455,7 @@
 template <class S, bool FROM_P, bool WANT_LL, bool TINY = false>
 __global__ __launch_bounds__(256, PLSA_WAVES) void k_row_pass(const int *__restrict__ indptr,
                                                   const int *__restrict__ colidx,
-                                                  const float *__restrict__ vals, int n,
+                                                  const float *__restrict__ vals, const int *__restrict__ sblk, int n,
                                                   const int *__restrict__ row_order,
                                                   const float *__restrict__ U,
                                                   const float *__restrict__ Vt,
@@ -424,7 +467,7 @@
                                                   const int *__restrict__ ritem_row,
                                                   const int *__restrict__ ritem_start, int rseg,
                                                   i64 n_ritems, float *__restrict__ rpartial, int xcd_rows) {
-    row_pass_body<S, FROM_P, WANT_LL, TINY>(indptr, colidx, vals, n, row_order, U, Vt, P, U_new, sw, norm_pdz_out, kp_rt, thresh,
+    row_pass_body<S, FROM_P, WANT_LL, TINY>(indptr, colidx, vals, sblk, n, row_order, U, Vt, P, U_new, sw, norm_pdz_out, kp_rt, thresh,
                                             ll_partials, ritem_row, ritem_start, rseg, n_ritems, rpartial, xcd_rows,
                                             blockIdx.x, gridDim.x);
 }
@@ -571,7 +614,7 @@
 __device__ __forceinline__ void col_pass_body(const int4 *__restrict__ item_rec, i64 n_items,
                                                   const int *__restrict__ xcd_lo,
                                                   const int *__restrict__ csc_row,
-                                                  const float *__restrict__ csc_val,
+                                                  const float *__restrict__ csc_val, int slot,
                                                   const int *__restrict__ csc_pos,
                                                   const float *__restrict__ U,
                                                   const float *__restrict__ Vt,
@@ -601,17 +644,15 @@
             const int w = rec.x, j0 = rec.y, j1 = rec.z;
             float4 vt[CH];
             load_row<S, true, PLSA_NT_STREAMS>(Vt + (i64)w * kp, li, kp, vt);
-            int d_n = (j0 + li < j1) ? ldi(csc_row + j0 + li) : 0;
-            float x_n = (!S::PACKED && j0 + li < j1) ? ldf(csc_val + j0 + li) : 0.f;
+            EntryCursor<S> es;
+            es.open(csc_row, csc_val, S::PACKED ? rec.w * slot : 0, j0, j1, li);
             int p_n = (FROM_P && j0 + li < j1) ? ldi(csc_pos + j0 + li) : 0;
             for (int jb = j0; jb < j1; jb += LPN) {
-                int d_l = d_n;
+                int d_l;
                 const int p_l = p_n;
-                float x_l = x_n;
-                if (S::PACKED) unpack_entry(d_l, x_l, csc_val, jb + li, j1);
+                float x_l;
+                es.take(csc_row, csc_val, jb, j1, li, d_l, x_l);
                 const int jn = jb + LPN + li;
-                d_n = jn < j1 ? ldi(csc_row + jn) : 0;
-                if (!S::PACKED) x_n = jn < j1 ? ldf(csc_val + jn) : 0.f;
                 if (FROM_P) p_n = jn < j1 ? ldi(csc_pos + jn) : 0;
                 if (sw) x_l *= sw[d_l];
                 const int cnt = min(LPN, j1 - jb);
@@ -636,7 +677,7 @@
 __global__ __launch_bounds__(256, PLSA_WAVES_COL) void k_col_pass(const int4 *__restrict__ item_rec, i64 n_items,
                                                   const int *__restrict__ xcd_lo,
                                                   const int *__restrict__ csc_row,
-                                                  const float *__restrict__ csc_val,
+                                                  const float *__restrict__ csc_val, int slot,
                                                   const int *__restrict__ csc_pos,
                                                   const float *__restrict__ U,
                                                   const float *__restrict__ Vt,
@@ -646,7 +687,7 @@
                                                   int xcd_split, double *__restrict__ chunk_sums,
                                                   unsigned long long *__restrict__ t_end) {
     extern __shared__ double scol[];
-    col_pass_body<S, FROM_P, TIMED, TINY>(item_rec, n_items, xcd_lo, csc_row, csc_val, csc_pos, U, Vt, P, sw, partial, kp_rt, thresh,
+    col_pass_body<S, FROM_P, TIMED, TINY>(item_rec, n_items, xcd_lo, csc_row, csc_val, slot, csc_pos, U, Vt, P, sw, partial, kp_rt, thresh,
                                           xcd_split, chunk_sums, t_end, scol, blockIdx.x, gridDim.x);
 }
 
@@ -1063,34 +1104,52 @@
     for (int o = 32; o > 0; o >>= 1) esc += __shfl_xor(esc, o, 64);
     if ((threadIdx.x & 63) == 0 && esc) atomicAdd(n_esc, (unsigned long long)esc);
 }
-__global__ __launch_bounds__(256) void k_pack_entries(const int *__restrict__ ids, const float *__restrict__ vals, i64 nnz,
-                                                      unsigned *__restrict__ packed, unsigned long long *__restrict__ n_esc) {
+__global__ __launch_bounds__(256) void k_pack_entries(const int *__restrict__ ids, const float *__restrict__ vals, i64 n_words,
+                                                      int lpn, const int *__restrict__ blk, const int *__restrict__ ptr,
+                                                      int n_owners, const int *__restrict__ item_start,
+                                                      const int *__restrict__ item_end, const int *__restrict__ item_row,
+                                                      int seg, int slot, unsigned *__restrict__ packed,
+                                                      unsigned long long *__restrict__ n_esc) {
     unsigned esc = 0;
-    for (i64 i = (i64)blockIdx.x * blockDim.x + threadIdx.x; i < nnz; i += (i64)gridDim.x * blockDim.x) {
-        const unsigned code = pack_code(vals[i]);
-        packed[i] = (unsigned)ids[i] | (code << 24);
-        esc += code == 0u;
+    const int block_words = plan::line_block(lpn);
+    for (i64 p = (i64)blockIdx.x * blockDim.x + threadIdx.x; p < n_words; p += (i64)gridDim.x * blockDim.x) {
+        int j0, j_end;
+        i64 word;
+        if (blk) {
+            const int b = (int)(p / block_words);
+            int lo = 0, hi = n_owners - 1;
+            while (lo < hi) {
+                const int mid = (int)(((i64)lo + hi + 1) >> 1);
+                if (blk[mid] <= b) lo = mid; else hi = mid - 1;
+            }
+            j0 = ptr[lo]; j_end = ptr[lo + 1];
+            word = p - (i64)blk[lo] * block_words;
+        } else {
+            const i64 it = p / slot;
+            j0 = item_start[it];
+            j_end = item_end ? item_end[it] : min(j0 + seg, ptr[item_row[it] + 1]);
+            word = p - it * slot;
+        }
+        const i64 rel = plan::line_rel(plan::line_pos_of_word(word, lpn), lpn);
+        unsigned e = 0u;
+        if (rel < (i64)(j_end - j0)) {
+            const i64 j = j0 + rel;
+            const unsigned code = pack_code(vals[j]);
+            e = (unsigned)ids[j] | (code << 24);
+            esc += code == 0u;
+        }
+        packed[p] = e;
     }
     add_escapes(esc, n_esc);
 }
 __global__ __launch_bounds__(256) void k_csc_gather(const int *__restrict__ pos, const int *__restrict__ rowidx,
                                                     const float *__restrict__ vals, i64 nnz, int *__restrict__ csc_row,
-                                                    float *__restrict__ csc_val, unsigned *__restrict__ packed,
-                                                    unsigned long long *__restrict__ n_esc) {
-    unsigned esc = 0;
+                                                    float *__restrict__ csc_val) {
     for (i64 i = (i64)blockIdx.x * blockDim.x + threadIdx.x; i < nnz; i += (i64)gridDim.x * blockDim.x) {
         const int p = pos[i];
-        const int r = rowidx[p];
-        const float v = vals[p];
-        csc_row[i] = r;
-        csc_val[i] = v;
-        if (packed) {
-            const unsigned code = pack_code(v);
-            packed[i] = (unsigned)r | (code << 24);
-            esc += code == 0u;
-        }
-    }
-    if (packed) add_escapes(esc, n_esc);
+        csc_row[i] = rowidx[p];
+        csc_val[i] = vals[p];
+    }
 }
 __global__ void k_item_counts(const int *__restrict__ colptr, int m, int seg, int *__restrict__ cnt) {
     const i64 c = (i64)blockIdx.x * blockDim.x + threadIdx.x;
diff --git a/enstop_amd/csrc/plsa_launch_plan.hpp b/enstop_amd/csrc/plsa_launch_plan.hpp
--- a/enstop_amd/csrc/plsa_launch_plan.hpp
+++ b/enstop_amd/csrc/plsa_launch_plan.hpp
@@ -73,6 +73,23 @@
 inline bool packed_ok(int64_t nnz, int64_t id_range, uint64_t escaped) {
     return nnz > 0 && id_range <= PACK_ID_RANGE && escaped * 16 <= (uint64_t)nnz;
 }
+
+constexpr int64_t LINE_MAX_WORDS = ((int64_t)1 << 31) - 1;
+constexpr int line_block(int lpn) { return 4 * lpn; }
+constexpr int64_t line_blocks(int64_t len, int lpn) { return (len + line_block(lpn) - 1) / line_block(lpn); }
+constexpr int line_slot(int seg, int lpn) { return (int)(line_blocks(seg, lpn) * line_block(lpn)); }
+struct LinePos { int64_t block; int lane, comp; };
+constexpr LinePos line_pos(int64_t rel, int lpn) {
+    return LinePos{rel / line_block(lpn), (int)(rel % line_block(lpn) % lpn), (int)(rel % line_block(lpn) / lpn)};
+}
+constexpr int64_t line_rel(const LinePos &p, int lpn) { return p.block * line_block(lpn) + (int64_t)p.comp * lpn + p.lane; }
+constexpr int64_t line_word(const LinePos &p, int lpn) { return p.block * line_block(lpn) + 4 * (int64_t)p.lane + p.comp; }
+constexpr LinePos line_pos_of_word(int64_t word, int lpn) {
+    return LinePos{word / line_block(lpn), (int)(word % line_block(lpn) / 4), (int)(word % 4)};
+}
+constexpr int64_t line_doc_words_bound(int64_t nnz, int64_t n, int lpn) { return nnz + n * (line_block(lpn) - 1); }
+constexpr int64_t line_item_words(int64_t n_items, int seg, int lpn) { return n_items * line_slot(seg, lpn); }
+constexpr bool line_stream_fits(int64_t words) { return words <= LINE_MAX_WORDS; }
 
 inline int grid_for(int64_t work, int per_block, int cap) {
     int64_t need = (work + per_block - 1) / per_block;
diff --git a/enstop_amd/csrc/plsa_member_kernels.hpp b/enstop_amd/csrc/plsa_member_kernels.hpp
--- a/enstop_amd/csrc/plsa_member_kernels.hpp
+++ b/enstop_amd/csrc/plsa_member_kernels.hpp
@@ -10,6 +10,7 @@
     const int4 *item_rec;
     const int *csc_row;
     const float *csc_val;
+    int slot;
     float *partial;
     double *chunk_sums;
     i64 n_items;
@@ -20,6 +21,7 @@
     int m, n_heavy, heavy_items, reduce_grid;
     const int *indptr, *colidx;
     const float *vals;
+    const int *sblk;
     const int *row_order, *ritem_row, *ritem_start, *ritem_first;
     float *rpartial;
     double *ll_partials, *ll_out;
@@ -38,7 +40,7 @@
     const MemberArgs &a = args[r];
     if (blockIdx.x >= (unsigned)a.row_grid) return;
     const int pu = (int)((cu >> r) & 1ull), pv = (int)((cv >> r) & 1ull);
-    row_pass_body<S, false, WANT_LL, TINY>(a.indptr, a.colidx, a.vals, a.n, a.row_order, a.U[pu], a.Vt[pv], nullptr, a.U[1 - pu],
+    row_pass_body<S, false, WANT_LL, TINY>(a.indptr, a.colidx, a.vals, a.sblk, a.n, a.row_order, a.U[pu], a.Vt[pv], nullptr, a.U[1 - pu],
                                            nullptr, nullptr, kp_rt, thresh, a.ll_partials, a.ritem_row, a.ritem_start, a.rseg,
                                            a.n_ritems, a.rpartial, 0, blockIdx.x, (unsigned)a.row_grid);
 }
@@ -71,7 +73,7 @@
     if (blockIdx.x >= (unsigned)a.n_chunks) return;
     const int pu = (int)((cu >> r) & 1ull), pv = (int)((cv >> r) & 1ull);
     const unsigned nblocks = min((unsigned)a.n_chunks, gridDim.x);
-    col_pass_body<S, false, false, TINY>(a.item_rec, a.n_items, nullptr, a.csc_row, a.csc_val, nullptr, a.U[pu], a.Vt[pv], nullptr,
+    col_pass_body<S, false, false, TINY>(a.item_rec, a.n_items, nullptr, a.csc_row, a.csc_val, a.slot, nullptr, a.U[pu], a.Vt[pv], nullptr,
                                          nullptr, a.partial, kp_rt, thresh, 0, a.chunk_sums, nullptr, scol, blockIdx.x, nblocks);
 }
 
diff --git a/enstop_amd/csrc/plsa_members.hpp b/enstop_amd/csrc/plsa_members.hpp
--- a/enstop_amd/csrc/plsa_members.hpp
+++ b/enstop_amd/csrc/plsa_members.hpp
@@ -72,6 +72,7 @@
     a.item_rec = l.item_rec;
     a.csc_row = l.csc_row;
     a.csc_val = l.csc_val;
+    a.slot = l.slot;
     a.partial = l.partial;
     a.chunk_sums = l.colsum_rows;
     a.n_items = l.n_items;
@@ -88,6 +89,7 @@
     a.indptr = r.indptr;
     a.colidx = r.colidx;
     a.vals = r.vals;
+    a.sblk = r.sblk;
     a.row_order = r.order;
     a.ritem_row = r.ritem_row;
     a.ritem_start = r.ritem_start;
diff --git a/enstop_amd/csrc/plsa_nmf.hpp b/enstop_amd/csrc/plsa_nmf.hpp
--- a/enstop_amd/csrc/plsa_nmf.hpp
+++ b/enstop_amd/csrc/plsa_nmf.hpp
@@ -45,7 +45,7 @@
         auto launch = [&](auto SS) {
             Scope s(c, "k_nmf_row_pass");
             hipLaunchKernelGGL((plsa::k_nmf_row_pass<decltype(SS)>), dim3(r.plan.grid), dim3(256), 0, c->ls, r.indptr, r.colidx,
-                               r.vals, n, r.order, W, Vt, hs, kp, iters, r.ritem_row, r.ritem_start, r.rseg, r.n_ritems, r.rpartial);
+                               r.vals, r.sblk, n, r.order, W, Vt, hs, kp, iters, r.ritem_row, r.ritem_start, r.rseg, r.n_ritems, r.rpartial);
         };
         if (r.packed) launch(plsa::Packed<Sh>{}); else launch(Sh{});
         if (r.items) {
@@ -69,7 +69,7 @@
         auto launch = [&](auto SS) {
             Scope s(c, "k_nmf_col_pass");
             hipLaunchKernelGGL((plsa::k_nmf_col_pass<decltype(SS)>), dim3(grid), dim3(256), 0, c->ls, l.item_rec, l.n_items,
-                               l.csc_row, l.csc_val, W, Vt, l.partial, c->kp);
+                               l.csc_row, l.csc_val, l.slot, W, Vt, l.partial, c->kp);
         };
         if (l.packed) launch(plsa::Packed<Sh>{}); else launch(Sh{});
     }));
diff --git a/enstop_amd/csrc/plsa_nmf_kernels.hpp b/enstop_amd/csrc/plsa_nmf_kernels.hpp
--- a/enstop_amd/csrc/plsa_nmf_kernels.hpp
+++ b/enstop_amd/csrc/plsa_nmf_kernels.hpp
@@ -58,19 +58,16 @@
 }
 
 template <class S, int UN>
-__device__ __forceinline__ void nmf_sweep(const int *__restrict__ ids, const float *__restrict__ vals, int j0, int j1,
+__device__ __forceinline__ void nmf_sweep(const int *__restrict__ ids, const float *__restrict__ vals, int sbase, int j0, int j1,
                                           int li, int kp, const float *table, const float4 (&own)[S::CH],
                                           float4 (&acc)[S::CH]) {
     constexpr int LPN = S::LPN;
-    int id_n = (j0 + li < j1) ? ldi(ids + j0 + li) : 0;
-    float x_n = (!S::PACKED && j0 + li < j1) ? ldf(vals + j0 + li) : 0.f;
+    EntryCursor<S> es;
+    es.open(ids, vals, sbase, j0, j1, li);
     for (int jb = j0; jb < j1; jb += LPN) {
-        int id_l = id_n;
-        float x_l = x_n;
-        if (S::PACKED) unpack_entry(id_l, x_l, vals, jb + li, j1);
-        const int jn = jb + LPN + li;
-        id_n = jn < j1 ? ldi(ids + jn) : 0;
-        if (!S::PACKED) x_n = jn < j1 ? ldf(vals + jn) : 0.f;
+        int id_l;
+        float x_l;
+        es.take(ids, vals, jb, j1, li, id_l, x_l);
         const int cnt = min(LPN, j1 - jb);
         int s0 = 0;
         for (; s0 + UN <= cnt; s0 += UN) nmf_batch<S, UN>(s0, id_l, x_l, li, kp, table, own, acc);
@@ -81,7 +78,7 @@
 
 template <class S>
 __global__ __launch_bounds__(256) void k_nmf_row_pass(const int *__restrict__ indptr, const int *__restrict__ colidx,
-                                                      const float *__restrict__ vals, int n,
+                                                      const float *__restrict__ vals, const int *__restrict__ sblk, int n,
                                                       const int *__restrict__ row_order, float *W,
                                                       const float *__restrict__ Vt, const float *__restrict__ h_sum,
                                                       int kp_rt, int iters, const int *__restrict__ ritem_row,
@@ -102,10 +99,11 @@
         const int j1 = items ? min(j0 + rseg, indptr[d + 1]) : indptr[d + 1];
         float4 w[CH], acc[CH];
         load_row<S, true>(W + (i64)d * kp, li, kp, w);
+        const int sbase = S::PACKED ? (items ? (int)r * row_item_slot<LPN>(rseg) : sblk[d] * (4 * LPN)) : 0;
         for (int it = 0; it < iters; ++it) {
 #pragma unroll
             for (int j = 0; j < CH; ++j) acc[j] = zero4();
-            nmf_sweep<S, S::UNR>(colidx, vals, j0, j1, li, kp, Vt, w, acc);
+            nmf_sweep<S, S::UNR>(colidx, vals, sbase, j0, j1, li, kp, Vt, w, acc);
             if (items) break;
 #pragma unroll
             for (int j = 0; j < CH; ++j) w[j] = S::ok(li, j, kp) ? nmf_scale(w[j], acc[j], hs[j]) : zero4();
@@ -153,7 +151,7 @@
 template <class S>
 __global__ __launch_bounds__(256) void k_nmf_col_pass(const int4 *__restrict__ item_rec, i64 n_items,
                                                       const int *__restrict__ csc_row, const float *__restrict__ csc_val,
-                                                      const float *__restrict__ W, const float *__restrict__ Vt,
+                                                      int slot, const float *__restrict__ W, const float *__restrict__ Vt,
                                                       float *__restrict__ partial, int kp_rt) {
     constexpr int LPN = S::LPN, CH = S::CH;
     constexpr int GPB = 256 / LPN;
@@ -166,7 +164,7 @@
         load_row<S, true>(Vt + (i64)rec.x * kp, li, kp, h);
 #pragma unroll
         for (int j = 0; j < CH; ++j) acc[j] = zero4();
-        nmf_sweep<S, S::UNR_COL>(csc_row, csc_val, rec.y, rec.z, li, kp, W, h, acc);
+        nmf_sweep<S, S::UNR_COL>(csc_row, csc_val, S::PACKED ? rec.w * slot : 0, rec.y, rec.z, li, kp, W, h, acc);
 #pragma unroll
         for (int j = 0; j < CH; ++j)
             if (S::ok(li, j, kp)) st4(partial + (i64)rec.w * kp + S::c4(li, j), acc[j]);
diff --git a/enstop_amd/csrc/plsa_structures.hpp b/enstop_amd/csrc/plsa_structures.hpp
--- a/enstop_amd/csrc/plsa_structures.hpp
+++ b/enstop_amd/csrc/plsa_structures.hpp
@@ -25,11 +25,14 @@
     c->row_lpn = sh.row_lpn; c->row_ch = sh.row_ch;
     if (c->row_lpn != prev_row_lpn) {
         c->ritems.invalidate();
+        c->pk_csr.invalidate();
         c->struct_row_lpn = c->row_lpn;
     }
     if (lpn != prev_lpn) {
         c->eitems.invalidate();
-        if (!c->seg_override) { c->csc.invalidate(); c->pk_csc.invalidate(); }
+        if (!c->seg_override) c->csc.invalidate();
+        c->pk_csc.reshape = c->seg_override && (c->pk_csc.valid || c->pk_csc.reshape);
+        c->pk_csc.invalidate();
         c->struct_lpn = lpn;
     }
 }
@@ -148,12 +151,12 @@
     return 0;
 }
 
-int packed_begin(plsa_ctx *c, plsa_ctx::PackedStream &s, i64 id_range, bool *pack) {
+int packed_begin(plsa_ctx *c, plsa_ctx::PackedStream &s, i64 id_range, i64 words_bound, bool *pack) {
     s.invalidate();
     s.ok = false;
-    *pack = c->packed && plsa::plan::packed_ok(c->nnz, id_range, 0);
+    s.reshape = false;
+    *pack = c->packed && plsa::plan::packed_ok(c->nnz, id_range, 0) && plsa::plan::line_stream_fits(words_bound);
     if (!*pack) return 0;
-    CHK(ensure(c, s.buf, sizeof(unsigned) * (size_t)c->nnz));
     CHK(ensure(c, c->pk_count, sizeof(unsigned long long)));
     HIPCHK(c, hipMemsetAsync(c->pk_count.p, 0, sizeof(unsigned long long), c->stream));
     return 0;
@@ -166,23 +169,62 @@
         HIPCHK(c, hipStreamSynchronize(c->stream));
     }
     s.ok = pack && plsa::plan::packed_ok(c->nnz, id_range, escaped);
-    if (!s.ok) s.buf.release();
+    if (!s.ok) { s.buf.release(); s.blk.release(); }
     s.valid = true;
     return 0;
 }
 
-int build_packed(plsa_ctx *c, plsa_ctx::PackedStream &s, const int *ids, const float *vals, i64 id_range) {
+int write_packed(plsa_ctx *c, plsa_ctx::PackedStream &s, const int *ids, const float *vals, int lpn, int seg, i64 n_items,
+                 const int *item_start, const int *item_end, const int *item_row) {
+    s.lpn = lpn; s.seg = seg;
+    const int block = plsa::plan::line_block(lpn), slot = seg > 0 ? plsa::plan::line_slot(seg, lpn) : 0;
+    auto pack = [&](const int *blk) {
+        CHK(ensure(c, s.buf, sizeof(unsigned) * (size_t)std::max<i64>(s.words, 1)));
+        if (s.words > 0)
+            hipLaunchKernelGGL(plsa::k_pack_entries, dim3(grid_for(c, s.words, 256)), dim3(256), 0, c->stream, ids, vals, s.words,
+                               lpn, blk, c->indptr, (int)c->n, item_start, item_end, item_row, seg, slot, s.buf.as<unsigned>(),
+                               c->pk_count.as<unsigned long long>());
+        return launch_check(c, "k_pack_entries");
+    };
+    if (seg > 0) {
+        s.words = plsa::plan::line_item_words(n_items, seg, lpn);
+        return pack(nullptr);
+    }
+    i64 n_blocks = 0;
+    return cut_items(c, c->indptr, c->n, block, s.blk, {}, &n_blocks, [&](int blocks) {
+        s.words = (i64)blocks * block;
+        return pack(s.blk.as<int>());
+    });
+}
+
+int build_packed_csr(plsa_ctx *c) {
+    plsa_ctx::PackedStream &s = c->pk_csr;
+    const bool items = c->ritems.use && c->ritems.n > 0;
+    const int lpn = c->row_lpn, seg = items ? c->ritems.seg : 0;
+    const i64 bound = items ? plsa::plan::line_item_words(c->ritems.n, seg, lpn) : plsa::plan::line_doc_words_bound(c->nnz, c->n, lpn);
     bool pack = false;
-    CHK(packed_begin(c, s, id_range, &pack));
-    if (pack) {
-        hipLaunchKernelGGL(plsa::k_pack_entries, dim3(grid_for(c, c->nnz, 256)), dim3(256), 0, c->stream,
-                           ids, vals, c->nnz, s.buf.as<unsigned>(), c->pk_count.as<unsigned long long>());
-        CHK(launch_check(c, "k_pack_entries"));
-    }
-    return packed_finish(c, s, id_range, pack);
-}
-
-int csc_order_entries(plsa_ctx *c, bool pack) {
+    CHK(packed_begin(c, s, c->m, bound, &pack));
+    if (pack)
+        CHK(write_packed(c, s, c->col, c->val, lpn, seg, c->ritems.n, items ? c->ritems.start.as<int>() : nullptr, nullptr,
+                         items ? c->ritems.row.as<int>() : nullptr));
+    return packed_finish(c, s, c->m, pack);
+}
+
+int write_packed_csc(plsa_ctx *c, bool pack) {
+    if (!pack) return 0;
+    return write_packed(c, c->pk_csc, c->csc.row.as<int>(), c->csc.val.as<float>(), c->lpn, c->csc.seg, c->csc.n_items,
+                        c->csc.item_start.as<int>(), c->csc.item_end.as<int>(), nullptr);
+}
+i64 packed_csc_words(const plsa_ctx *c, i64 n_items_bound) { return plsa::plan::line_item_words(n_items_bound, c->csc.seg, c->lpn); }
+
+int build_packed_csc(plsa_ctx *c) {
+    bool pack = false;
+    CHK(packed_begin(c, c->pk_csc, c->n, packed_csc_words(c, c->csc.n_items), &pack));
+    CHK(write_packed_csc(c, pack));
+    return packed_finish(c, c->pk_csc, c->n, pack);
+}
+
+int csc_order_entries(plsa_ctx *c) {
     plsa_ctx::Csc &s = c->csc;
     const i64 nnz = c->nnz, m = c->m;
     if (nnz <= 0) {
@@ -199,8 +241,7 @@
     hipLaunchKernelGGL(plsa::k_colptr_from_sorted, dim3((unsigned)((m + 256) / 256)), dim3(256), 0, c->stream,
                        c->tmp0.as<int>(), nnz, (int)m, s.colptr.as<int>());
     hipLaunchKernelGGL(plsa::k_csc_gather, dim3(grid_for(c, nnz, 256)), dim3(256), 0, c->stream,
-                       s.pos.as<int>(), c->rowidx.ids.as<int>(), c->val, nnz, s.row.as<int>(), s.val.as<float>(),
-                       pack ? c->pk_csc.buf.as<unsigned>() : nullptr, pack ? c->pk_count.as<unsigned long long>() : nullptr);
+                       s.pos.as<int>(), c->rowidx.ids.as<int>(), c->val, nnz, s.row.as<int>(), s.val.as<float>());
     return launch_check(c, "k_csc_gather");
 }
 
@@ -257,7 +298,10 @@
 }
 
 int ensure_csc(plsa_ctx *c) {
-    if (c->csc.valid) return 0;
+    if (c->csc.valid) {
+        if (!c->pk_csc.valid && c->pk_csc.reshape) CHK(build_packed_csc(c));
+        return 0;
+    }
     CHK(ensure_rowidx(c));
     c->csc.seg = plsa::plan::col_item_len(c->nnz, c->prop.multiProcessorCount, c->lpn, c->seg_override);
     const i64 nnz = c->nnz, m = c->m;
@@ -268,9 +312,10 @@
     CHK(ensure(c, c->tmp0, sizeof(int) * (size_t)std::max<i64>(nnz, m + 1)));
     CHK(ensure(c, c->tmp1, sizeof(int) * (size_t)nnz));
     bool pack = false;
-    CHK(packed_begin(c, c->pk_csc, c->n, &pack));
-    CHK(csc_order_entries(c, pack));
+    CHK(packed_begin(c, c->pk_csc, c->n, packed_csc_words(c, nnz / std::max(c->csc.seg, 1) + m), &pack));
+    CHK(csc_order_entries(c));
     CHK(csc_items_in_visiting_order(c));
+    CHK(write_packed_csc(c, pack));
     CHK(csc_item_records(c));
     CHK(csc_heavy_list(c));
     if (!pack) HIPCHK(c, hipStreamSynchronize(c->stream));
@@ -280,14 +325,17 @@
 }
 
 int ensure_packed_csr(plsa_ctx *c) {
-    if (!c->packed || c->pk_csr.valid) return 0;
-    return build_packed(c, c->pk_csr, c->col, c->val, c->m);
+    if (!c->packed) return 0;
+    CHK(ensure_ritems(c));
+    const int seg = c->ritems.use && c->ritems.n > 0 ? c->ritems.seg : 0;
+    if (c->pk_csr.valid && (!c->pk_csr.ok || (c->pk_csr.lpn == c->row_lpn && c->pk_csr.seg == seg))) return 0;
+    return build_packed_csr(c);
 }
 
 int ensure_packed_csc(plsa_ctx *c) {
     CHK(ensure_csc(c));
     if (!c->packed || c->pk_csc.valid) return 0;
-    return build_packed(c, c->pk_csc, c->csc.row.as<int>(), c->csc.val.as<float>(), c->n);
+    return build_packed_csc(c);
 }
 
 int balance_set_lo(plsa_ctx *c, int n_chunks) {
```
